# imkaywu/MVSKit

Measured on AMD Instinct MI355X. Metric: patches/s (propagate+optim iteration), 12-view 1080p, higher is better.
Workload: dtype f32

## Files before the change

### mvskit_amd/csrc/mvs_engine.cpp

```cpp
#include <dlfcn.h>

#include <cmath>
#include <cstring>

#include "mvs_engine_impl.h"

using namespace mvseng;

static_assert(sizeof(mvs_patch) == sizeof(DPatch), "mvs_patch and DPatch must be the same bytes");
static_assert((MVS_LISTCAP == 16 || MVS_LISTCAP == 32 || MVS_LISTCAP == 64) && MVS_LISTCAP <= MVS_MAXI && MVS_MAX_IMAGES == MVS_MAXI, "limits out of sync");

namespace mvseng {

thread_local std::string g_err;

Roctx& roctx() {
    static Roctx r;
    static bool tried = false;
    if (tried) return r;
    tried = true;
    void* h = nullptr;
    const char* names[] = {"libroctx64.so", "libroctx64.so.4", "/opt/rocm/lib/libroctx64.so.4"};
    for (const char* n : names) if (!h) h = dlopen(n, RTLD_NOW | RTLD_NOLOAD);
    for (const char* n : names) if (!h) h = dlopen(n, RTLD_NOW | RTLD_LOCAL);
    if (!h) return r;
    r.push = reinterpret_cast<int (*)(const char*)>(dlsym(h, "roctxRangePushA"));
    r.pop = reinterpret_cast<int (*)()>(dlsym(h, "roctxRangePop"));
    if (!r.push || !r.pop) { r.push = nullptr; r.pop = nullptr; }
    return r;
}

RefineSel refine_sel(const mvs_engine* e) {
    return RefineSel{e->refiner.mode == MVS_REFINE_CONVERGED ? 1 : 0, e->refiner.max_evals, e->refiner.xtol};
}

DParams current_params(mvs_engine* e) {
    DParams p = e->prm;
    p.views = e->dviews.p;
    p.pyr32 = e->pyr_narrow ? e->pyr.p : nullptr;
    p.pool = e->pool.p;
    p.pool_n = e->pool_n;
    p.total_cells = e->total_cells;
    p.csr_start = e->start.p; p.csr_cnt = e->cnt_alive.p; p.csr_key = e->key.p; p.csr_id32 = e->id32.p;
    p.vcsr_start = e->vstart.p; p.vcsr_cnt = e->vcnt_alive.p; p.vcsr_id32 = e->vid32.p;
    p.dpgrid = e->dpgrid.p;
    p.geo = e->geo_valid ? e->geo.p : nullptr;
    p.geo_ref = e->geo_valid ? e->geo_ref.p : nullptr;
    return p;
}

bool want_vgrid(const mvs_engine* e) { return e->prm.depth >= 2 && e->prm.enable_check; }

int need_state(const mvs_engine* e, Need need, const char* who) {
    if (!e) { g_err = std::string(who) + ": no engine"; return MVS_ERR_ARG; }
    if (need >= NEED_VIEWS && !e->have_views) { g_err = std::string(who) + ": views not set"; return MVS_ERR_STATE; }
    if (need >= NEED_IDLE && e->staged) { g_err = std::string(who) + ": a pass is waiting for its commit"; return MVS_ERR_STATE; }
    return MVS_OK;
}

int scan_total(mvs_engine* e, const int32_t* flags, int32_t* base, int32_t* scan, int64_t n, int64_t* count) {
    mvsk_exclusive_scan(flags, base, n, scan, e->stream);
    int32_t total = 0;
    if (int r = read_back(e, base + n, &total)) return r;
    HIPCHK(hipGetLastError());
    *count = total;
    return MVS_OK;
}

}

namespace {

void derive_params(mvs_engine* e) {
    const mvs_config& c = e->cfg;
    DParams& p = e->prm;
    p.nviews = c.nviews; p.level = c.level; p.csize = c.csize; p.wsize = c.wsize; p.wsz = c.wsize * c.wsize;
    p.minImageNum = c.minImageNum;
    p.tau = std::min(c.minImageNum * 2, c.nviews);
    p.max_propag = c.max_propag;
    p.cap = c.max_propag * c.csize * c.csize;
    p.depth = c.depth; p.enable_check = c.enable_check; p.view_propagation = c.view_propagation ? 1 : 0;
    p.seed = c.seed; p.refine_steps = c.refine_steps; p.rd0 = c.refine_rd0; p.ra0 = c.refine_ra0;
    p.nccThreshold = c.nccThreshold;
    p.nccThresholdBefore = c.nccThreshold - 0.3f;
    volatile float a0 = (float)(60.0f * M_PI / 180.0f), a1 = (float)(60.0f * M_PI / 180.0f);
    volatile double amin = (double)c.maxAngleThreshold, amax = (double)a1;
    volatile float typo = (float)(120.0f / M_PI * 180.0f);
    volatile double d120 = 120.0f * M_PI / 180.0f, d10 = 10.0f * M_PI / 180.0f;
    p.cosAngle0 = cosf(a0);
    p.cosAngle1 = cosf(a1);
    p.cosMinAngle = (float)cos(amin);
    p.cosMaxAngle = (float)cos(amax);
    p.cosNeighborTypo = cosf(typo);
    p.cosNeighbor120 = (float)cos(d120);
    p.sortThreshold = (float)(1.0f - cos(d10));
    p.ascaleConst = (float)(M_PI / 48.0f);
    p.inv_sz = 1.0f / (float)(c.wsize * c.wsize);
    p.inv_3sz = 1.0f / (float)(3 * c.wsize * c.wsize);
    p.neighborThreshold = 0.5f; p.neighborThreshold1 = 1.0f;
    p.quadThreshold = c.quadThreshold;
    p.list_n = std::min<int>(MVS_LISTCAP, c.nviews);
    p.gram_ld = (p.list_n + 15) / 16 * 16;
}

void invert3(const float* P, float* Minv) {
    double a = P[0], b = P[1], c = P[2], d = P[4], e = P[5], f = P[6], g = P[8], h = P[9], i = P[10];
    double A = e * i - f * h, B = -(d * i - f * g), C = d * h - e * g;
    double det = a * A + b * B + c * C;
    double inv[9] = {A, -(b * i - c * h), b * f - c * e, B, a * i - c * g, -(a * f - c * d), C, -(a * h - b * g), a * e - b * d};
    for (int k = 0; k < 9; ++k) Minv[k] = (float)(inv[k] / det);
}
inline float hfma(float a, float b, float c) { return __builtin_fmaf(a, b, c); }
inline float hdot3(const float* a, const float* b) { return hfma(a[2], b[2], hfma(a[1], b[1], a[0] * b[0])); }
inline float hdot4(const float* a, const float* b) { return hfma(a[3], b[3], hfma(a[2], b[2], hfma(a[1], b[1], a[0] * b[0]))); }
inline void hcross(const float* a, const float* b, float* o) {
    o[0] = a[1] * b[2] - a[2] * b[1]; o[1] = a[2] * b[0] - a[0] * b[2]; o[2] = a[0] * b[1] - a[1] * b[0];
}

void setup_camera(const mvs_engine* e, DView& vw, const float* P0) {
    const int maxLevel = e->cfg.level + 3;
    for (int k = 0; k < 12; ++k) vw.P[0][k] = P0[k];
    for (int l = 1; l < maxLevel; ++l) {
        for (int k = 0; k < 12; ++k) vw.P[l][k] = vw.P[l - 1][k];
        for (int k = 0; k < 8; ++k) vw.P[l][k] /= 2.0f;
    }
    invert3(vw.P[e->cfg.level], vw.Minv);
    const float* r2 = &vw.P[0][8];
    const float n = sqrtf(hdot3(r2, r2));
    for (int k = 0; k < 4; ++k) vw.oaxis[k] = r2[k] / n;
    {
        const float* P = vw.P[0];
        double a = P[0], b = P[1], c = P[2], d = P[4], ee = P[5], f = P[6], g = P[8], h = P[9], i = P[10];
        double A = ee * i - f * h, B = -(d * i - f * g), C = d * h - ee * g;
        double det = a * A + b * B + c * C;
        double inv[9] = {A, -(b * i - c * h), b * f - c * ee, B, a * i - c * g, -(a * f - c * d), C, -(a * h - b * g), a * ee - b * d};
        double q[3] = {P[3], P[7], P[11]};
        vw.center[0] = (float)(-(inv[0] * q[0] + inv[1] * q[1] + inv[2] * q[2]) / det);
        vw.center[1] = (float)(-(inv[3] * q[0] + inv[4] * q[1] + inv[5] * q[2]) / det);
        vw.center[2] = (float)(-(inv[6] * q[0] + inv[7] * q[1] + inv[8] * q[2]) / det);
        vw.center[3] = 1.0f;
    }
    for (int k = 0; k < 3; ++k) vw.zaxis[k] = vw.oaxis[k];
    float xa[3] = {vw.P[0][0], vw.P[0][1], vw.P[0][2]};
    hcross(vw.zaxis, xa, vw.yaxis);
    const float yn = sqrtf(hdot3(vw.yaxis, vw.yaxis));
    for (int k = 0; k < 3; ++k) vw.yaxis[k] /= yn;
    hcross(vw.yaxis, vw.zaxis, vw.xaxis);
    const float x4[4] = {vw.xaxis[0], vw.xaxis[1], vw.xaxis[2], 0.0f}, y4[4] = {vw.yaxis[0], vw.yaxis[1], vw.yaxis[2], 0.0f};
    vw.ipscale = hdot4(&vw.P[0][0], x4) + hdot4(&vw.P[0][4], y4);
}

}

extern "C" {

const char* mvs_last_error(void) { return g_err.c_str(); }

int mvs_list_cap(void) { return MVS_LISTCAP; }
int mvs_patch_bytes(void) { return (int)sizeof(mvs_patch); }

int mvs_device_count(void) {
    int n = 0;
    if (hipGetDeviceCount(&n) != hipSuccess) return 0;
    return n;
}

void mvs_default_refiner(mvs_refiner* r) {
    if (!r) return;
    r->mode = MVS_REFINE_HALVING; r->max_evals = 500; r->xtol = 1e-4f;
}

int mvs_engine_set_refiner(mvs_engine* e, const mvs_refiner* r) {
    if (!e || !r) { g_err = "mvs_engine_set_refiner: null argument"; return MVS_ERR_ARG; }
    if ((r->mode != MVS_REFINE_HALVING && r->mode != MVS_REFINE_CONVERGED) || r->max_evals < 5 || r->max_evals > 4096 ||
        !std::isfinite(r->xtol) || !(r->xtol > 0.0f)) {
        g_err = "mvs_engine_set_refiner: unknown mode, max_evals outside 5..4096, or xtol not finite and > 0";
        return MVS_ERR_ARG;
    }
    e->refiner = *r;
    return MVS_OK;
}

void mvs_default_config(mvs_config* c) {
    memset(c, 0, sizeof *c);
    c->level = 1; c->csize = 2; c->wsize = 7; c->minImageNum = 3; c->max_propag = 2;
    c->nccThreshold = 0.7f; c->maxAngleThreshold = (float)(10.0f * M_PI / 180.0f); c->quadThreshold = 2.5f;
    c->depth = 1; c->seed = 1; c->refine_steps = 6; c->refine_rd0 = 4.0f; c->refine_ra0 = 4.0f; c->enable_check = 1;
    c->view_begin = 0; c->view_stride = 1; c->device = 0; c->max_patches = 0;
}

int mvs_engine_create(const mvs_config* cfg, mvs_engine** out) {
    if (!cfg || !out) { g_err = "mvs_engine_create: null argument"; return MVS_ERR_ARG; }
    if (cfg->shard_count > 1 && (cfg->shard_index < 0 || cfg->shard_index >= cfg->shard_count)) { g_err = "mvs_engine_create: bad shard_index"; return MVS_ERR_ARG; }
    if (cfg->nviews < 1 || cfg->nviews > MVS_MAXVIEWS || cfg->wsize < 1 || cfg->wsize > 7 || cfg->csize < 1 || cfg->level < 0 ||
        cfg->level > 4 || cfg->max_propag < 1 || cfg->max_propag > 16 || cfg->max_propag * cfg->csize * cfg->csize > MVS_CAPMAX ||
        cfg->view_stride < 1 || cfg->view_begin < 0 || cfg->minImageNum < 1 ||
        std::min(cfg->minImageNum * 2, cfg->nviews) > 16 ) {
        g_err = "mvs_engine_create: configuration out of range (nviews <= 64, wsize <= 7, min(2 minImageNum, nviews) <= 16, max_propag*csize^2 <= 32)";
        return MVS_ERR_ARG;
    }
    int ndev = 0;
    if (hipGetDeviceCount(&ndev) != hipSuccess || ndev < 1) { g_err = "mvs_engine_create: no HIP device (the engine has no CPU path)"; return MVS_ERR_NO_DEVICE; }
    if (cfg->device < 0 || cfg->device >= ndev) { g_err = "mvs_engine_create: bad device ordinal"; return MVS_ERR_ARG; }
    HIPCHK(hipSetDevice(cfg->device));
    mvs_engine* e = new mvs_engine();
    e->cfg = *cfg;
    derive_params(e);
    hipError_t he = hipStreamCreate(&e->stream);
    if (he != hipSuccess) { g_err = std::string("hipStreamCreate: ") + hipGetErrorString(he); delete e; return MVS_ERR_HIP; }
    for (auto& ev : e->ev) (void)hipEventCreate(&ev);
    for (auto& ev : e->fev) (void)hipEventCreate(&ev);
    if (e->misc.ensure(misc::words) || e->counters.ensure(MVS_COUNTER_SLOTS) || e->error_flag.ensure(1)) { delete e; return MVS_ERR_HIP; }
    (void)hipMemset(e->misc.p, 0, misc::words * sizeof(unsigned long long));
    (void)hipMemset(e->error_flag.p, 0, sizeof(int32_t));
    *out = e;
    return MVS_OK;
}

int mvs_engine_destroy(mvs_engine* e) {
    if (!e) return MVS_OK;
    (void)hipSetDevice(e->cfg.device);
    (void)hipStreamSynchronize(e->stream);
    (void)mvs_engine_comm_release(e);
    for (auto& ev : e->ev) if (ev) (void)hipEventDestroy(ev);
    for (auto& ev : e->fev) if (ev) (void)hipEventDestroy(ev);
    (void)hipStreamDestroy(e->stream);
    delete e;
    return MVS_OK;
}

int mvs_engine_set_views(mvs_engine* e, int nviews, const mvs_view_desc* views) {
    if (!e || !views || nviews != e->cfg.nviews) { g_err = "mvs_engine_set_views: nviews must equal the configured number of views"; return MVS_ERR_ARG; }
    HIPCHK(hipSetDevice(e->cfg.device));
    hipStream_t st = e->stream;
    Range rg("mvs:set_views (upload + pyramids)");
    e->mask_bufs.clear();
    e->have_views = false;
    const int maxLevel = e->cfg.level + 3;
    e->hviews.assign(nviews, DView{});
    int cell_base = 0;
    size_t max_bytes = 0;
    for (int v = 0; v < nviews; ++v) {
        if (views[v].width < 8 || views[v].height < 8 || !views[v].rgb) { g_err = "mvs_engine_set_views: bad view"; return MVS_ERR_ARG; }
        max_bytes = std::max(max_bytes, (size_t)views[v].width * views[v].height * 3);
    }
    if (int r = e->tmp_bytes.ensure((int64_t)max_bytes)) return r;
    std::vector<uint64_t> level_off((size_t)nviews * maxLevel);
    uint64_t pyr_bytes = 0;
    bool narrow = true;
    for (int v = 0; v < nviews; ++v) {
        DView& vw = e->hviews[v];
        vw.W[0] = views[v].width; vw.H[0] = views[v].height;
        for (int l = 1; l < maxLevel; ++l) { vw.W[l] = vw.W[l - 1] / 2; vw.H[l] = vw.H[l - 1] / 2; }
        for (int l = 0; l < maxLevel; ++l) {
            level_off[(size_t)v * maxLevel + l] = pyr_bytes;
            pyr_bytes += (std::max<uint64_t>((uint64_t)vw.W[l] * vw.H[l], 1) * 4 + 255) / 256 * 256;
        }
        if ((int64_t)vw.W[0] * 4 >= (1 << 24) || vw.H[0] >= (1 << 24)) narrow = false;
    }
    if (pyr_bytes >= (1ull << 32)) narrow = false;
    if (int r = e->pyr.ensure((int64_t)pyr_bytes)) return r;
    e->pyr_narrow = narrow;
    for (int v = 0; v < nviews; ++v) {
        DView& vw = e->hviews[v];
        setup_camera(e, vw, views[v].P);
        const size_t n0 = (size_t)vw.W[0] * vw.H[0];
        HIPCHK(hipMemcpyAsync(e->tmp_bytes.p, views[v].rgb, n0 * 3, hipMemcpyHostToDevice, st));
        for (int l = 0; l < maxLevel; ++l) {
            const uint64_t off = level_off[(size_t)v * maxLevel + l];
            uint32_t* buf = reinterpret_cast<uint32_t*>(e->pyr.p + off);
            vw.img[l] = buf;
            vw.img_off[l] = (uint32_t)off;
            if (l == 0) mvsk_rgb_to_rgba(e->tmp_bytes.p, buf, (int64_t)n0, st);
            else mvsk_pyr_down(vw.img[l - 1], vw.W[l - 1], vw.H[l - 1], buf, vw.W[l], vw.H[l], st);
        }
        vw.mask = nullptr;
        if (views[v].mask) {
            HIPCHK(hipStreamSynchronize(st));
            uint8_t* prev = nullptr;
            for (int l = 0; l <= e->cfg.level; ++l) {
                e->mask_bufs.emplace_back();
                if (int r = e->mask_bufs.back().ensure(std::max<int64_t>((int64_t)vw.W[l] * vw.H[l], 1))) return r;
                uint8_t* m = e->mask_bufs.back().p;
                if (l == 0) {
                    HIPCHK(hipMemcpyAsync(m, views[v].mask, n0, hipMemcpyHostToDevice, st));
                    mvsk_mask_binarise(m, (int64_t)n0, st);
                } else mvsk_mask_down(prev, vw.W[l - 1], vw.H[l - 1], m, vw.W[l], vw.H[l], st);
                prev = m;
            }
            vw.mask = prev;
        }
        HIPCHK(hipStreamSynchronize(st));
        vw.gh = (vw.H[e->cfg.level] + e->cfg.csize - 1) / e->cfg.csize;
        vw.gw = (vw.W[e->cfg.level] + e->cfg.csize - 1) / e->cfg.csize;
        vw.cell_base = cell_base;
        cell_base += vw.gw * vw.gh;
    }
    e->total_cells = cell_base;
    if (int r = e->dviews.ensure(nviews)) return r;
    HIPCHK(hipMemcpyAsync(e->dviews.p, e->hviews.data(), sizeof(DView) * nviews, hipMemcpyHostToDevice, st));
    const int64_t nc = e->total_cells;
    if (e->cnt.ensure(nc + 2) || e->start.ensure(nc + 2) || e->cursor.ensure(nc + 2) || e->vcnt.ensure(nc + 2) || e->vstart.ensure(nc + 2) ||
        e->vcursor.ensure(nc + 2) || e->start_raw.ensure(nc + 2) || e->dpgrid.ensure(nc + 2) || e->best.ensure(nc + 2) || e->cnt_alive.ensure(nc + 2) || e->vcnt_alive.ensure(nc + 2))
        return MVS_ERR_HIP;
    int64_t pool_cap = e->cfg.max_patches > 0 ? e->cfg.max_patches : 4 * nc;
    if (e->cfg.max_patches <= 0) {
        size_t free_b = 0, total_b = 0;
        if (hipMemGetInfo(&free_b, &total_b) == hipSuccess && total_b > 0) {
            pool_cap = std::max<int64_t>(std::min<int64_t>(pool_cap, (int64_t)(total_b / 6 / sizeof(DPatch))), std::min<int64_t>(pool_cap, nc));
            const double per_patch = 2.5 * (double)sizeof(DPatch) + 17.0;
            const int64_t fit = (int64_t)(0.6 * (double)free_b / per_patch);
            if (fit < pool_cap) pool_cap = std::max<int64_t>(fit, std::min<int64_t>(pool_cap, nc / 4 + 1024));
        }
    }
    e->ids.headroom = e->key.headroom = e->id32.headroom = e->id32_raw.headroom = e->vid32.headroom = true;
    e->geo.headroom = e->geo_ref.headroom = true;
    if (e->pool.ensure(pool_cap) || e->pool_alt.ensure(pool_cap) || e->kill.ensure(pool_cap) || e->kill_cnt.ensure(pool_cap + 2) || e->kill_base.ensure(pool_cap + 2)) return MVS_ERR_HIP;
    HIPCHK(hipMemsetAsync(e->kill.p, 0, (size_t)pool_cap, st));
    int64_t njobs_max = 0;
    for (int v = 0; v < nviews; ++v) njobs_max += (int64_t)((e->hviews[v].gw + 1) / 2) * e->hviews[v].gh;
    const int maxstage = (e->prm.view_propagation ? 3 : 2) * e->prm.cap * e->prm.max_propag;
    if (e->job_stage.ensure(njobs_max * maxstage) || e->job_nstage.ensure(njobs_max + 2) || e->job_cnt.ensure(njobs_max + misc::job_list_pad) ||
        e->job_base_scan.ensure(njobs_max + misc::job_list_pad) || e->job_list.ensure(std::max<int64_t>(njobs_max, 16)))
        return MVS_ERR_HIP;
    const int64_t scan_n = std::max<int64_t>(std::max<int64_t>(nc, pool_cap), njobs_max);
    if (e->scan_tmp.ensure(scan_n / 256 + 4096)) return MVS_ERR_HIP;
    if (e->big_tables.ensure((int64_t)256 * 16384) || e->retry_jobs.ensure(std::max<int64_t>(njobs_max, 16))) return MVS_ERR_HIP;
    if (e->uf_parent.ensure(pool_cap) || e->uf_size.ensure(pool_cap) || e->dirty.ensure((nc + 31) / 32 + 1) || e->fstat_buf.ensure(fstat::words)) return MVS_ERR_HIP;
    if (e->staging.ensure(std::max<int64_t>(pool_cap / 2, 1024))) return MVS_ERR_HIP;
    if (e->tmp_rec_out.ensure(16)) return MVS_ERR_HIP;
    HIPCHK(hipStreamSynchronize(st));
    e->pool_n = 0;
    e->have_views = true;
    e->staged = false;
    return MVS_OK;
}

int mvs_engine_grid_dims(mvs_engine* e, int view, int* gw, int* gh) {
    if (!e || !e->have_views || view < 0 || view >= e->cfg.nviews) { g_err = "mvs_engine_grid_dims: bad view / views not set"; return MVS_ERR_STATE; }
    if (gw) *gw = e->hviews[view].gw;
    if (gh) *gh = e->hviews[view].gh;
    return MVS_OK;
}

int mvs_engine_get_pyramid(mvs_engine* e, int view, int level, uint8_t* rgb_out, int* W, int* H) {
    if (!e || !e->have_views || view < 0 || view >= e->cfg.nviews || level < 0 || level >= e->cfg.level + 3) { g_err = "mvs_engine_get_pyramid: bad argument"; return MVS_ERR_ARG; }
    HIPCHK(hipSetDevice(e->cfg.device));
    const DView& vw = e->hviews[view];
    if (W) *W = vw.W[level];
    if (H) *H = vw.H[level];
    if (!rgb_out) return MVS_OK;
    const int64_t n = (int64_t)vw.W[level] * vw.H[level];
    if (int r = e->tmp_bytes.ensure(n * 3)) return r;
    mvsk_rgba_to_rgb(vw.img[level], e->tmp_bytes.p, n, e->stream);
    HIPCHK(hipMemcpyAsync(rgb_out, e->tmp_bytes.p, (size_t)n * 3, hipMemcpyDeviceToHost, e->stream));
    HIPCHK(hipStreamSynchronize(e->stream));
    return MVS_OK;
}

int mvs_engine_set_thresholds(mvs_engine* e, float ncc, float before, int depth) {
    if (!e) return MVS_ERR_ARG;
    e->prm.nccThreshold = ncc; e->prm.nccThresholdBefore = before; e->prm.depth = depth;
    return MVS_OK;
}
int mvs_engine_get_thresholds(mvs_engine* e, float* ncc, float* before, int* depth) {
    if (!e) return MVS_ERR_ARG;
    if (ncc) *ncc = e->prm.nccThreshold;
    if (before) *before = e->prm.nccThresholdBefore;
    if (depth) *depth = e->prm.depth;
    return MVS_OK;
}
int mvs_engine_update_threshold(mvs_engine* e) {
    if (!e) return MVS_ERR_ARG;
    e->prm.nccThreshold -= 0.05f; e->prm.nccThresholdBefore -= 0.05f; ++e->prm.depth;
    return MVS_OK;
}

int mvs_engine_upload_patches(mvs_engine* e, int64_t n, const mvs_patch* patches) {
    if (!e || !e->have_views) { g_err = "mvs_engine_upload_patches: views not set"; return MVS_ERR_STATE; }
    if (n < 0 || (n > 0 && !patches)) return MVS_ERR_ARG;
    if (e->staged) { g_err = "mvs_engine_upload_patches: a pass is waiting for its commit"; return MVS_ERR_STATE; }
    HIPCHK(hipSetDevice(e->cfg.device));
    Range rg("mvs:upload_patches");
    std::vector<mvs_patch> recs;
    recs.reserve((size_t)n);
    for (int64_t i = 0; i < n; ++i) {
        mvs_patch p = patches[i];
        p.nimages = std::min(p.nimages, MVS_LISTCAP);
        if (p.nimages <= 0) continue;
        memset(p.images + p.nimages, 0, sizeof p.images - (size_t)p.nimages);
        p.nvimages = 0;
        memset(p.vimages, 0, sizeof p.vimages);
        p.tmp = std::max(0.0f, p.ncc - e->prm.nccThreshold) * p.nimages;
        p.flags = 1;
        p.id = 0;
        recs.push_back(p);
    }
    if (e->pool_n + (int64_t)recs.size() > e->pool.cap) { g_err = "mvs_engine_upload_patches: patch pool capacity exceeded (raise mvs_config.max_patches)"; return MVS_ERR_CAPACITY; }
    if (!recs.empty()) HIPCHK(hipMemcpyAsync(e->pool.p + e->pool_n, recs.data(), recs.size() * sizeof(mvs_patch), hipMemcpyHostToDevice, e->stream));
    HIPCHK(hipStreamSynchronize(e->stream));
    e->pool_n += (int64_t)recs.size();
    e->ncc_dirty = true;
    return MVS_OK;
}

int mvs_engine_reserve(mvs_engine* e, int64_t list_entries) {
    if (!e || !e->have_views || list_entries < 0) { g_err = "mvs_engine_reserve: views not set, or a negative size"; return MVS_ERR_ARG; }
    HIPCHK(hipSetDevice(e->cfg.device));
    int64_t n = list_entries > 0 ? list_entries : e->total_cells * (int64_t)(e->cfg.max_propag * e->cfg.csize * e->cfg.csize);
    auto take = [&](auto& buf, int64_t want) -> int {
        const int64_t before = buf.cap;
        if (int r = buf.ensure(want)) return r;
        if (buf.cap != before && hipMemsetAsync(buf.p, 0, (size_t)buf.cap * sizeof(*buf.p), e->stream) != hipSuccess) { (void)hipGetLastError(); return MVS_ERR_HIP; }
        return MVS_OK;
    };
    if (take(e->ids, n + 16) || take(e->key, n + 16) || take(e->id32, n + 16) || take(e->id32_raw, n + 16) || take(e->vid32, n + 16)) return MVS_ERR_HIP;
    HIPCHK(hipStreamSynchronize(e->stream));
    return MVS_OK;
}

int mvs_engine_clear_patches(mvs_engine* e) {
    if (!e) return MVS_ERR_ARG;
    HIPCHK(hipSetDevice(e->cfg.device));
    if (e->kill.p) HIPCHK(hipMemsetAsync(e->kill.p, 0, (size_t)e->kill.cap, e->stream));
    e->pool_n = 0; e->staged = false; e->counted = false;
    return MVS_OK;
}

int mvs_engine_num_patches(mvs_engine* e, int64_t* n_alive) {
    if (!e || !n_alive) return MVS_ERR_ARG;
    HIPCHK(hipSetDevice(e->cfg.device));
    return count_pool(e, Count::alive, n_alive);
}

int mvs_engine_download_patches(mvs_engine* e, int64_t cap, mvs_patch* out, int64_t* n) {
    if (!e || !n) return MVS_ERR_ARG;
    int64_t alive = 0;
    if (int r = mvs_engine_num_patches(e, &alive)) return r;
    *n = alive;
    if (!out || alive == 0) return MVS_OK;
    const int64_t m = std::min(cap, alive);
    if (int r = e->tmp_rec_out.ensure(alive)) return r;
    mvsk_alive_gather(e->pool.p, e->pool_n, e->kill_base.p, e->tmp_rec_out.p, alive, e->stream);
    HIPCHK(hipMemcpyAsync(out, e->tmp_rec_out.p, (size_t)m * sizeof(mvs_patch), hipMemcpyDeviceToHost, e->stream));
    HIPCHK(hipStreamSynchronize(e->stream));
    return MVS_OK;
}

int mvs_engine_sweep_pairs(mvs_engine* e, int64_t out[6]) {
    if (!e || !out) return MVS_ERR_ARG;
    for (int k = 0; k < 6; ++k) out[k] = e->sweep_pairs[k];
    return MVS_OK;
}

int mvs_engine_sweep_repeats(mvs_engine* e, int64_t out[2]) {
    if (!e || !out) return MVS_ERR_ARG;
    for (int k = 0; k < 2; ++k) out[k] = e->sweep_repeats[k];
    return MVS_OK;
}

int mvs_engine_sweep_kernels(mvs_engine* e, int64_t out[2]) {
    if (!e || !out) return MVS_ERR_ARG;
    for (int k = 0; k < 2; ++k) out[k] = e->sweep_kernels[k];
    return MVS_OK;
}

int mvs_engine_sampler_launches(mvs_engine* e, int64_t out[4]) {
    if (!e || !out) return MVS_ERR_ARG;
    for (int k = 0; k < 4; ++k) out[k] = e->sampler_launches[k];
    return MVS_OK;
}

int mvs_engine_last_timing(mvs_engine* e, mvs_timing* t) {
    if (!e || !t) return MVS_ERR_ARG;
    *t = e->timing;
    return MVS_OK;
}

int mvs_engine_depth_normal_map(mvs_engine* e, int view, int kind, float* depth, float* normal, int32_t* ids) {
    if (!e || !e->have_views || view < 0 || view >= e->cfg.nviews || kind < 0 || kind > 1) { g_err = "mvs_engine_depth_normal_map: bad argument"; return MVS_ERR_ARG; }
    HIPCHK(hipSetDevice(e->cfg.device));
    hipStream_t st = e->stream;
    const DView& vw = e->hviews[view];
    const int ncells = vw.gw * vw.gh;
    const DParams p = current_params(e);
    const unsigned long long* sel = nullptr;
    if (kind == 0) {
        HIPCHK(hipMemsetAsync(e->dpgrid.p, 0xff, (size_t)e->total_cells * sizeof(unsigned long long), st));
        mvsk_depth_maps(p, e->dpgrid.p, nullptr, st);
        sel = e->dpgrid.p + vw.cell_base;
    } else {
        HIPCHK(hipMemsetAsync(e->best.p, 0, (size_t)ncells * sizeof(unsigned long long), st));
        mvsk_best_ncc_map(p, view, e->best.p, st);
        sel = e->best.p;
    }
    if (e->tmp_f_out.ensure((int64_t)ncells * 4) || e->tmp_i.ensure(ncells)) return MVS_ERR_HIP;
    mvsk_map_extract(p, view, kind, sel, e->tmp_f_out.p, e->tmp_f_out.p + ncells, e->tmp_i.p, ncells, st);
    if (depth) HIPCHK(hipMemcpyAsync(depth, e->tmp_f_out.p, (size_t)ncells * sizeof(float), hipMemcpyDeviceToHost, st));
    if (normal) HIPCHK(hipMemcpyAsync(normal, e->tmp_f_out.p + ncells, (size_t)ncells * 3 * sizeof(float), hipMemcpyDeviceToHost, st));
    if (ids) HIPCHK(hipMemcpyAsync(ids, e->tmp_i.p, (size_t)ncells * sizeof(int32_t), hipMemcpyDeviceToHost, st));
    HIPCHK(hipStreamSynchronize(st));
    return MVS_OK;
}

int mvs_engine_probe(mvs_engine* e, int op, int64_t n, const mvs_patch* in_rec, const float* in_f, mvs_patch* out_rec, float* out_f, int32_t* out_i) {
    if (!e || !e->have_views || n < 0 || op < 0 || op > 6) { g_err = "mvs_engine_probe: bad argument / views not set"; return MVS_ERR_ARG; }
    const RefineSel rs = refine_sel(e);
    if (op == MVS_PROBE_REFINE_X && !rs.simplex) { g_err = "mvs_engine_probe: MVS_PROBE_REFINE_X needs the CONVERGED refiner"; return MVS_ERR_STATE; }
    if (n == 0) return MVS_OK;
    HIPCHK(hipSetDevice(e->cfg.device));
    hipStream_t st = e->stream;
    if (op == MVS_PROBE_POSTPROCESS && e->prm.depth > 0) if (int r = build_index(e, nullptr)) return r;
    const int64_t nf_out = op == MVS_PROBE_MATH ? 5 * n : ((op == MVS_PROBE_REFINE || op == MVS_PROBE_REFINE_X) && rs.simplex ? 4 * n : n);
    if (e->tmp_rec_in.ensure(n) || e->tmp_rec_out.ensure(n) || e->tmp_f_in.ensure(n) || e->tmp_f_out.ensure(nf_out) || e->tmp_i.ensure(n + 1)) return MVS_ERR_HIP;
    if (op == MVS_PROBE_MATH) {
        if (!in_f || !out_f) return MVS_ERR_ARG;
        HIPCHK(hipMemcpyAsync(e->tmp_f_in.p, in_f, (size_t)n * sizeof(float), hipMemcpyHostToDevice, st));
    } else {
        if (!in_rec) return MVS_ERR_ARG;
        HIPCHK(hipMemcpyAsync(e->tmp_rec_in.p, in_rec, (size_t)n * sizeof(mvs_patch), hipMemcpyHostToDevice, st));
    }
    HIPCHK(hipMemsetAsync(e->tmp_i.p, 0, (size_t)(n + 1) * sizeof(int32_t), st));
    const DParams p = current_params(e);
    const KernelVariant probe_kernel = mvsk_probe(p, op, n, e->tmp_rec_in.p, e->tmp_f_in.p, e->tmp_rec_out.p, e->tmp_f_out.p, e->tmp_i.p, rs, st);
    if (probe_kernel.launched) e->sampler_launches[probe_kernel.narrow ? 3 : 2] += 1;
    if (out_rec && (op == MVS_PROBE_PREPROCESS || op == MVS_PROBE_REFINE || op == MVS_PROBE_POSTPROCESS || op == MVS_PROBE_REFINE_X))
        HIPCHK(hipMemcpyAsync(out_rec, e->tmp_rec_out.p, (size_t)n * sizeof(mvs_patch), hipMemcpyDeviceToHost, st));
    if (out_f && (op == MVS_PROBE_NCC || op == MVS_PROBE_COST || op == MVS_PROBE_MATH || op == MVS_PROBE_REFINE_X))
        HIPCHK(hipMemcpyAsync(out_f, e->tmp_f_out.p, (size_t)nf_out * sizeof(float), hipMemcpyDeviceToHost, st));
    if (out_i) HIPCHK(hipMemcpyAsync(out_i, e->tmp_i.p, (size_t)n * sizeof(int32_t), hipMemcpyDeviceToHost, st));
    HIPCHK(hipStreamSynchronize(st));
    HIPCHK(hipGetLastError());
    return MVS_OK;
}

}
```

### mvskit_amd/csrc/mvs_engine_impl.h

```cpp
#pragma once
#include <hip/hip_runtime.h>
#include <rccl/rccl.h>

#include <algorithm>
#include <cstdint>
#include <string>
#include <vector>

#include "mvskit_engine.h"
#include "mvs_kernels.h"
#include "mvs_types.h"

namespace mvseng {
extern thread_local std::string g_err;
}

#define HIPCHK(expr)                                                                                       \
    do {                                                                                                   \
        hipError_t _e = (expr);                                                                            \
        if (_e != hipSuccess) {                                                                            \
            mvseng::g_err = std::string(#expr) + ": " + hipGetErrorString(_e);                             \
            return MVS_ERR_HIP;                                                                            \
        }                                                                                                  \
    } while (0)

#define MVS_XCHG_WORDS 5

namespace mvseng {

template <typename T> struct DevBuf {
    T* p = nullptr;
    int64_t cap = 0;
    bool headroom = false;
    DevBuf() = default;
    DevBuf(const DevBuf&) = delete;
    DevBuf(DevBuf&& o) noexcept : p(o.p), cap(o.cap), headroom(o.headroom) { o.p = nullptr; o.cap = 0; }
    ~DevBuf() { release(); }
    void swap(DevBuf& o) { std::swap(p, o.p); std::swap(cap, o.cap); }
    int ensure(int64_t n) {
        if (n <= cap) return MVS_OK;
        const int64_t exact = std::max<int64_t>(n, 16);
        int64_t want = (p && headroom) ? exact + exact / 2 : exact;
        T* q = nullptr;
        hipError_t e = hipMalloc((void**)&q, (size_t)want * sizeof(T));
        if (e != hipSuccess && want > exact) { (void)hipGetLastError(); want = exact; e = hipMalloc((void**)&q, (size_t)want * sizeof(T)); }
        if (e != hipSuccess && p) {
            (void)hipGetLastError();
            (void)hipFree(p); p = nullptr; cap = 0;
            e = hipMalloc((void**)&q, (size_t)want * sizeof(T));
        }
        if (e != hipSuccess) { (void)hipGetLastError(); g_err = std::string("hipMalloc: ") + hipGetErrorString(e); return MVS_ERR_HIP; }
        if (p) (void)hipFree(p);
        p = q; cap = want;
        return MVS_OK;
    }
    void release() { if (p) (void)hipFree(p); p = nullptr; cap = 0; }
};

namespace misc {
constexpr int stage_counter = 0;
constexpr int fill_evals = 1;
constexpr int neighbor_retry = 4;
constexpr int sweep_retry = 5;
constexpr int geo_bad = 6;
constexpr int group_edges = 7;
constexpr int trim_parts = 8;
constexpr int trim_nparts = 256;
constexpr int sweep_cursors = (trim_parts + trim_nparts + 15) / 16 * 16;
constexpr int sweep_cursor_words = MVS_SWEEP_QUEUES * MVS_SWEEP_CURSOR_STRIDE * (int)sizeof(uint32_t) / (int)sizeof(unsigned long long);
constexpr int sweep_list_bounds = sweep_cursors + sweep_cursor_words;
constexpr int sweep_list_bound_words = (MVS_SWEEP_QUEUES + 1 + 1) / 2;
constexpr int words = sweep_list_bounds + sweep_list_bound_words;
constexpr int64_t job_list_pad = 1024 + 2;
}
namespace fstat {
constexpr int neighbor_parts = 0;
constexpr int neighbor_cycles = 4096;
constexpr int exact_evals = 4112;
constexpr int words = exact_evals + 2048;
}

struct Rccl {
    void* h = nullptr;
    ncclResult_t (*GetUniqueId)(ncclUniqueId*) = nullptr;
    ncclResult_t (*CommInitRank)(ncclComm_t*, int, ncclUniqueId, int) = nullptr;
    ncclResult_t (*CommDestroy)(ncclComm_t) = nullptr;
    ncclResult_t (*CommCount)(const ncclComm_t, int*) = nullptr;
    ncclResult_t (*CommUserRank)(const ncclComm_t, int*) = nullptr;
    ncclResult_t (*AllGather)(const void*, void*, size_t, ncclDataType_t, ncclComm_t, hipStream_t) = nullptr;
    ncclResult_t (*Broadcast)(const void*, void*, size_t, ncclDataType_t, int, ncclComm_t, hipStream_t) = nullptr;
    ncclResult_t (*GroupStart)() = nullptr;
    ncclResult_t (*GroupEnd)() = nullptr;
    const char* (*GetErrorString)(ncclResult_t) = nullptr;
    bool ok = false;
};
Rccl& rccl();

struct Roctx {
    int (*push)(const char*) = nullptr;
    int (*pop)() = nullptr;
};
Roctx& roctx();
struct Range {
    bool on;
    explicit Range(const char* name) : on(roctx().push != nullptr) { if (on) roctx().push(name); }
    ~Range() { if (on) roctx().pop(); }
    Range(const Range&) = delete;
    Range& operator=(const Range&) = delete;
};

}

using mvseng::DevBuf;
struct mvs_engine {
    mvs_config cfg{};
    mvs_refiner refiner{MVS_REFINE_HALVING, 500, 1e-4f};
    DParams prm{};
    hipStream_t stream = nullptr;
    bool have_views = false;
    std::vector<DView> hviews;
    DevBuf<DView> dviews;
    DevBuf<uint8_t> pyr;
    bool pyr_narrow = false;
    std::vector<DevBuf<uint8_t>> mask_bufs;
    int total_cells = 0;
    DevBuf<DPatch> pool, pool_alt;
    DevBuf<uint8_t> kill;
    int64_t pool_n = 0;
    bool ncc_dirty = false;
    DevBuf<int32_t> cnt, cursor, vcnt, vcursor;
    DevBuf<csr_off_t> start, vstart;
    DevBuf<csr_off_t> start_raw;
    DevBuf<int32_t> id32_raw;
    DevBuf<int64_t> scan_tmp;
    DevBuf<unsigned long long> ids;
    DevBuf<ListKey> key;
    DevBuf<int32_t> id32, vid32;
    DevBuf<int32_t> uf_parent, uf_size;
    DevBuf<int32_t> group_edges;
    DevBuf<int32_t> cnt_alive, vcnt_alive;
    DevBuf<unsigned long long> dpgrid, best;
    DevBuf<uint32_t> dirty;
    bool dirty_marked = false;
    DevBuf<float4> geo;
    DevBuf<uint8_t> geo_ref;
    bool geo_valid = false;
    bool lists_dense[2] = {false, false};
    DevBuf<DPatch> staging;
    DevBuf<int32_t> job_stage, job_nstage, job_cnt, job_base_scan, kill_cnt, kill_base;
    DevBuf<unsigned long long> misc;
    DevBuf<DCounters> counters;
    DevBuf<int32_t> error_flag;
    DevBuf<int32_t> big_tables, retry_jobs;
    DevBuf<int32_t> job_list;
    int64_t sweep_pairs[6] = {0, 0, 0, 0, 0, 0};
    int64_t sweep_repeats[2] = {0, 0};
    int64_t sweep_kernels[2] = {0, 0};
    int64_t sampler_launches[4] = {0, 0, 0, 0};
    int64_t retried_cells = 0;
    int64_t pass_retried = 0;
    SweepArgs sa{};
    bool staged = false;
    bool counted = false;
    int64_t n_new = 0, n_kill = 0;
    std::vector<int32_t> h_per_view;
    DevBuf<DPatch> tmp_rec_in, tmp_rec_out;
    DevBuf<float> tmp_f_in, tmp_f_out;
    DevBuf<int32_t> tmp_i;
    DevBuf<uint8_t> tmp_bytes;
    hipEvent_t ev[6] = {nullptr, nullptr, nullptr, nullptr, nullptr, nullptr};
    mvs_timing timing{};
    mvs_filter_stats fstats{};
    int64_t fstats_exchange_bytes = 0;
    DevBuf<unsigned long long> fstat_buf;
    hipEvent_t fev[10] = {nullptr, nullptr, nullptr, nullptr, nullptr, nullptr, nullptr, nullptr, nullptr, nullptr};
    ncclComm_t comm = nullptr;
    bool comm_owned = false;
    int comm_rank = 0, comm_world = 1;
    DevBuf<int64_t> comm_counts;
    DevBuf<int32_t> comm_kill_ids;
    int pass_status = MVS_OK;
    std::string pass_error;
    bool fault_fired = false;
};

namespace mvseng {

RefineSel refine_sel(const mvs_engine* e);
DParams current_params(mvs_engine* e);
bool want_vgrid(const mvs_engine* e);
enum Need { NEED_ENGINE, NEED_VIEWS, NEED_IDLE };
int need_state(const mvs_engine* e, Need need, const char* who);
int scan_total(mvs_engine* e, const int32_t* flags, int32_t* base, int32_t* scan, int64_t n, int64_t* count);

int build_list(mvs_engine* e, bool vgrid, bool trim, bool unordered = false);
int build_depth(mvs_engine* e);
int build_index(mvs_engine* e, unsigned long long* trimmed_out);
enum class Count { alive, kills, apply_kills };
int count_pool(mvs_engine* e, Count what, int64_t* total);
int ensure_counts(mvs_engine* e);
int compact_pool(mvs_engine* e);
void discard_pass(mvs_engine* e);

template <typename T> int read_back(mvs_engine* e, const T* dev, T* host) {
    HIPCHK(hipMemcpyAsync(host, dev, sizeof(T), hipMemcpyDeviceToHost, e->stream));
    HIPCHK(hipStreamSynchronize(e->stream));
    return MVS_OK;
}

template <typename Apply> int commit_pool(mvs_engine* e, Apply&& apply) {
    hipStream_t st = e->stream;
    HIPCHK(hipEventRecord(e->ev[2], st));
    int64_t n_new = 0;
    if (int r = apply(&n_new)) return r;
    e->pool_n += n_new;
    if (int r = compact_pool(e)) return r;
    HIPCHK(hipEventRecord(e->ev[3], st));
    HIPCHK(hipStreamSynchronize(st));
    float ms = 0.0f;
    (void)hipEventElapsedTime(&ms, e->ev[2], e->ev[3]);
    e->timing.commit_ms = ms;
    e->staged = false; e->counted = false;
    return MVS_OK;
}

template <typename Blocks> ncclResult_t broadcast_blocks(mvs_engine* e, Blocks&& blocks) {
    const Rccl& R = rccl();
    ncclResult_t first = R.GroupStart();
    for (int r = 0; r < e->comm_world && first == ncclSuccess; ++r)
        blocks(r, [&](void* p, int64_t n, ncclDataType_t type) {
            if (n > 0 && first == ncclSuccess) first = R.Broadcast(p, p, (size_t)n, type, r, e->comm, e->stream);
        });
    const ncclResult_t end = R.GroupEnd();
    return first == ncclSuccess ? end : first;
}

struct MapsBufs {
    MapsArgs args{};
    int64_t total_pix = 0, max_pix = 0;
    DevBuf<int32_t> ids;
    DevBuf<float> pts;
    DevBuf<unsigned long long> agree;
    DevBuf<int32_t> flag, base, scan;
    DevBuf<float> maps;
    DevBuf<uint8_t> flag8;
    DevBuf<mvs_fused_point> recs;
};
int maps_args(const mvs_maps_config* c, const char* who);
int maps_state(const mvs_engine* e, const mvs_maps_config* c, const char* who);
int64_t maps_npix(const mvs_engine* e, int v);
int render_all(mvs_engine* e, const mvs_maps_config* c, MapsBufs& b);
int render_usable(mvs_engine* e, const mvs_maps_config* c, MapsBufs& b);

}
```

### mvskit_amd/csrc/mvs_engine_pass.cpp

```cpp
#include <climits>
#include <cstdio>
#include <cstdlib>
#include <cstring>

#include "mvs_engine_impl.h"

using namespace mvseng;

namespace mvseng {

int build_list(mvs_engine* e, bool vgrid, bool trim, bool unordered) {
    hipStream_t st = e->stream;
    const int64_t nc = e->total_cells;
    DParams p = current_params(e);
    DevBuf<int32_t>& cnt = vgrid ? e->vcnt : e->cnt;
    DevBuf<csr_off_t>& start = vgrid ? e->vstart : e->start;
    DevBuf<int32_t>& cursor = vgrid ? e->vcursor : e->cursor;
    DevBuf<unsigned long long>& ids = e->ids;
    DevBuf<int32_t>& id32 = vgrid ? e->vid32 : e->id32;
    DevBuf<int32_t>& cnt_alive = vgrid ? e->vcnt_alive : e->cnt_alive;
    HIPCHK(hipMemsetAsync(cnt.p, 0, (size_t)(nc + 1) * sizeof(int32_t), st));
    mvsk_index_count(p, vgrid ? nullptr : cnt.p, vgrid ? cnt.p : nullptr, nullptr, st);
    const bool direct = unordered && !trim;
    DevBuf<csr_off_t>& raw = e->start_raw;
    csr_off_t* const first_scan = direct ? start.p : raw.p;
    mvsk_exclusive_scan_off(cnt.p, first_scan, nc, reinterpret_cast<csr_off_t*>(e->scan_tmp.p), st);
    csr_off_t tot64 = 0;
    if (int r = read_back(e, first_scan + nc, &tot64)) return r;
    const int64_t tot = (int64_t)tot64;
    if (!unordered) { if (int r = ids.ensure(tot + 16)) return r; }
    if (!vgrid && !unordered) { if (int r = e->key.ensure(tot + 16)) return r; }
    if (int r = id32.ensure(tot + 16)) return r;
    p = current_params(e);
    HIPCHK(hipMemsetAsync(cursor.p, 0, (size_t)(nc + 1) * sizeof(int32_t), st));
    if (direct) {
        mvsk_index_fill_direct(p, vgrid ? 1 : 0, start.p, cursor.p, id32.p, st);
        cnt.swap(cnt_alive);
        e->lists_dense[vgrid ? 1 : 0] = true;
        return MVS_OK;
    }
    if (int r = e->id32_raw.ensure(tot + 16)) return r;
    mvsk_index_fill(p, vgrid ? 1 : 0, raw.p, cursor.p, ids.p, st);
    mvsk_index_sort_trim(p, raw.p, ids.p, trim ? 1 : 0, e->misc.p + misc::trim_parts, st);
    mvsk_index_finalize(p, vgrid ? 1 : 0, raw.p, ids.p, e->id32_raw.p, cnt_alive.p, st);
    mvsk_exclusive_scan_off(cnt_alive.p, start.p, nc, reinterpret_cast<csr_off_t*>(e->scan_tmp.p), st);
    mvsk_index_pack(p, raw.p, start.p, cnt_alive.p, ids.p, e->id32_raw.p, vgrid ? nullptr : e->key.p, id32.p, st);
    e->lists_dense[vgrid ? 1 : 0] = true;
    return MVS_OK;
}
int build_depth(mvs_engine* e) {
    const DParams p = current_params(e);
    HIPCHK(hipMemsetAsync(e->dpgrid.p, 0xff, (size_t)e->total_cells * sizeof(unsigned long long), e->stream));
    mvsk_depth_maps(p, e->dpgrid.p, nullptr, e->stream);
    return MVS_OK;
}
int build_index(mvs_engine* e, unsigned long long* trimmed_out) {
    hipStream_t st = e->stream;
    const DParams p = current_params(e);
    HIPCHK(hipMemsetAsync(e->misc.p + misc::fill_evals, 0, 2 * sizeof(unsigned long long), st));
    HIPCHK(hipMemsetAsync(e->misc.p + misc::trim_parts, 0, misc::trim_nparts * sizeof(unsigned long long), st));
    mvsk_fill_ncc(p, e->misc.p + misc::fill_evals, st);
    e->ncc_dirty = false;
    if (int r = build_list(e, false, true)) return r;
    if (want_vgrid(e)) if (int r = build_list(e, true, false, true)) return r;
    if (int r = build_depth(e)) return r;
    if (trimmed_out) {
        unsigned long long part[misc::trim_nparts];
        HIPCHK(hipMemcpyAsync(part, e->misc.p + misc::trim_parts, sizeof part, hipMemcpyDeviceToHost, st));
        HIPCHK(hipStreamSynchronize(st));
        *trimmed_out = 0;
        for (unsigned long long v : part) *trimmed_out += v;
    }
    HIPCHK(hipGetLastError());
    return MVS_OK;
}

int count_pool(mvs_engine* e, Count what, int64_t* total) {
    hipStream_t st = e->stream;
    *total = 0;
    if (e->pool_n == 0) return MVS_OK;
    if (what == Count::alive) mvsk_alive_count(e->pool.p, e->pool_n, e->kill_cnt.p, st);
    else mvsk_kill_count(e->kill.p, e->pool_n, e->kill_cnt.p, st);
    mvsk_exclusive_scan(e->kill_cnt.p, e->kill_base.p, e->pool_n, reinterpret_cast<int32_t*>(e->scan_tmp.p), st);
    int32_t n = 0;
    HIPCHK(hipMemcpyAsync(&n, e->kill_base.p + e->pool_n, sizeof n, hipMemcpyDeviceToHost, st));
    if (what == Count::apply_kills) mvsk_apply_kill_flags(e->pool.p, e->kill.p, e->pool_n, st);
    HIPCHK(hipStreamSynchronize(st));
    *total = n;
    return MVS_OK;
}

int ensure_counts(mvs_engine* e) {
    if (e->counted) return MVS_OK;
    hipStream_t st = e->stream;
    const int64_t nj = e->sa.njobs;
    e->n_new = 0; e->n_kill = 0;
    e->h_per_view.assign(e->cfg.nviews, 0);
    if (nj > 0) {
        mvsk_commit_count(e->sa, e->job_cnt.p, st);
        mvsk_exclusive_scan(e->job_cnt.p, e->job_base_scan.p, nj, reinterpret_cast<int32_t*>(e->scan_tmp.p), st);
        std::vector<int32_t> bounds(e->sa.nsweep_views + 1);
        for (int s = 0; s < e->sa.nsweep_views; ++s)
            HIPCHK(hipMemcpyAsync(&bounds[s], e->job_base_scan.p + e->sa.job_base[s], sizeof(int32_t), hipMemcpyDeviceToHost, st));
        HIPCHK(hipMemcpyAsync(&bounds[e->sa.nsweep_views], e->job_base_scan.p + nj, sizeof(int32_t), hipMemcpyDeviceToHost, st));
        HIPCHK(hipStreamSynchronize(st));
        e->n_new = bounds[e->sa.nsweep_views];
        for (int s = 0; s < e->sa.nsweep_views; ++s) e->h_per_view[e->sa.sweep_views[s]] = bounds[s + 1] - bounds[s];
    }
    if (int r = count_pool(e, Count::kills, &e->n_kill)) return r;
    e->counted = true;
    return MVS_OK;
}

int compact_pool(mvs_engine* e) {
    int64_t alive = 0;
    if (int r = count_pool(e, Count::alive, &alive)) return r;
    if (alive == e->pool_n) return MVS_OK;
    mvsk_alive_gather(e->pool.p, e->pool_n, e->kill_base.p, e->pool_alt.p, e->pool_alt.cap, e->stream);
    e->pool.swap(e->pool_alt);
    e->pool_n = alive;
    return MVS_OK;
}

void discard_pass(mvs_engine* e) {
    if (e->kill.p && e->pool_n > 0) (void)hipMemsetAsync(e->kill.p, 0, (size_t)e->pool_n, e->stream);
    (void)hipStreamSynchronize(e->stream);
    e->staged = false; e->counted = false;
}

}

namespace {

template <typename C> void add_counters(mvs_counters& a, const C& b) {
    a.candidates += b.candidates; a.prefiltered += b.prefiltered; a.patches += b.patches; a.fail0 += b.fail0; a.fail1 += b.fail1;
    a.inserted += b.inserted; a.replaced += b.replaced; a.evals += b.evals; a.view_evals += b.view_evals; a.trimmed += b.trimmed;
}

}

extern "C" {

static int pass_impl(mvs_engine* e, int iter, int pass, mvs_counters* out);
int mvs_engine_pass(mvs_engine* e, int iter, int pass, mvs_counters* out) {
    const int r = pass_impl(e, iter, pass, out);
    if (e) { e->pass_status = r; e->pass_error = r ? g_err : std::string(); }
    return r;
}
static int pass_impl(mvs_engine* e, int iter, int pass, mvs_counters* out) {
    if (!e || !e->have_views) { g_err = "mvs_engine_pass: views not set"; return MVS_ERR_STATE; }
    if (e->staged) { g_err = "mvs_engine_pass: the previous pass was not committed"; return MVS_ERR_STATE; }
    HIPCHK(hipSetDevice(e->cfg.device));
    hipStream_t st = e->stream;
    HIPCHK(hipEventRecord(e->ev[0], st));
    unsigned long long trimmed = 0;
    {
        Range rg("mvs:index");
        if (int r = build_index(e, &trimmed)) return r;
    }
    SweepArgs& a = e->sa;
    memset(&a, 0, sizeof a);
    a.iter = iter; a.inc = (iter % 2 == 0) ? 1 : -1; a.colour = pass & 1;
    int64_t nj = 0;
    const bool ranged = e->cfg.shard_count > 1;
    for (int v = ranged ? 0 : e->cfg.view_begin; v < e->cfg.nviews; v += ranged ? 1 : e->cfg.view_stride) {
        a.sweep_views[a.nsweep_views] = v;
        a.job_base[a.nsweep_views] = (int32_t)nj;
        ++a.nsweep_views;
        nj += (int64_t)((e->hviews[v].gw + 1) / 2) * e->hviews[v].gh;
    }
    a.njobs = nj;
    a.job_lo = 0; a.job_hi = nj;
    if (ranged) {
        const int split_mode = getenv("MVS_SPLIT_PROXY") ? atoi(getenv("MVS_SPLIT_PROXY")) : 2;
        const int N = e->cfg.shard_count, R = e->cfg.shard_index;
        std::vector<int32_t> cuts(N + 1, -1);
        int64_t total_work = 0;
        if (split_mode > 0 && nj > 0) {
            const DParams p0 = current_params(e);
            int shift = 0;
            while ((((int64_t)3 * e->prm.cap * e->prm.max_propag * 32 * nj) >> shift) + nj >= (int64_t)INT32_MAX) ++shift;
            mvsk_job_work(p0, a, split_mode, shift, e->job_cnt.p, st);
            mvsk_exclusive_scan(e->job_cnt.p, e->job_base_scan.p, nj, reinterpret_cast<int32_t*>(e->scan_tmp.p), st);
            if (int r = e->tmp_i.ensure(N + 1)) return r;
            HIPCHK(hipMemsetAsync(e->tmp_i.p, 0xff, (size_t)(N + 1) * sizeof(int32_t), st));
            mvsk_job_cuts(e->job_base_scan.p, nj, N, e->tmp_i.p, st);
            int32_t tw = 0;
            HIPCHK(hipMemcpyAsync(cuts.data(), e->tmp_i.p, (size_t)(N + 1) * sizeof(int32_t), hipMemcpyDeviceToHost, st));
            HIPCHK(hipMemcpyAsync(&tw, e->job_base_scan.p + nj, sizeof tw, hipMemcpyDeviceToHost, st));
            HIPCHK(hipStreamSynchronize(st));
            total_work = tw;
        }
        cuts[0] = 0; cuts[N] = (int32_t)nj;
        for (int r = 1; r < N; ++r) {
            if (total_work <= 0 || cuts[r] < 0) cuts[r] = (int32_t)(nj * r / N);
            cuts[r] = std::max(cuts[r], cuts[r - 1]);
        }
        a.job_lo = cuts[R];
        a.job_hi = cuts[R + 1];
    }
    a.staging = e->staging.p; a.staging_cap = e->staging.cap;
    a.stage_counter = e->misc.p + misc::stage_counter;
    a.job_stage = e->job_stage.p; a.job_nstage = e->job_nstage.p;
    a.maxstage = (e->prm.view_propagation ? 3 : 2) * e->prm.cap * e->prm.max_propag;
    a.kill = e->kill.p;
    a.counters = e->counters.p;
    a.error_flag = e->error_flag.p;
    if (want_vgrid(e)) {
        if (int r = e->big_tables.ensure((int64_t)256 * 16384)) return r;
        if (int r = e->retry_jobs.ensure(std::max<int64_t>(nj, 16))) return r;
    }
    a.big_tables = e->big_tables.p; a.retry_jobs = e->retry_jobs.p; a.nretry = reinterpret_cast<int32_t*>(e->misc.p + misc::sweep_retry);
    HIPCHK(hipMemsetAsync(e->misc.p + misc::sweep_retry, 0, sizeof(unsigned long long), st));
    HIPCHK(hipMemsetAsync(e->misc.p + misc::stage_counter, 0, sizeof(unsigned long long), st));
    a.cursors = reinterpret_cast<uint32_t*>(e->misc.p + misc::sweep_cursors);
    HIPCHK(hipMemsetAsync(e->misc.p + misc::sweep_cursors, 0, (misc::sweep_cursor_words + misc::sweep_list_bound_words) * sizeof(unsigned long long), st));
    HIPCHK(hipMemsetAsync(e->counters.p, 0, MVS_COUNTER_SLOTS * sizeof(DCounters), st));
    HIPCHK(hipMemsetAsync(e->error_flag.p, 0, sizeof(int32_t), st));
    const DParams p = current_params(e);
    const RefineSel rs = refine_sel(e);
    if (int r = e->job_list.ensure(std::max<int64_t>(nj, 16))) return r;
    if (e->job_cnt.ensure(nj + misc::job_list_pad) || e->job_base_scan.ensure(nj + misc::job_list_pad)) return MVS_ERR_HIP;
    int32_t* list_bounds = reinterpret_cast<int32_t*>(e->misc.p + misc::sweep_list_bounds);
    a.job_list = e->job_list.p; a.list_bounds = list_bounds;
    mvsk_job_list(p, a, e->job_cnt.p, e->job_base_scan.p, reinterpret_cast<int32_t*>(e->scan_tmp.p), e->job_list.p, list_bounds, st);
    HIPCHK(hipEventRecord(e->ev[1], st));
    Range rg_sweep(pass & 1 ? "mvs:sweep colour 1" : "mvs:sweep colour 0");
    const KernelVariant sweep_kernel = mvsk_sweep(p, a, rs, st);
    if (sweep_kernel.launched) { e->sweep_kernels[sweep_kernel.full_window ? 1 : 0] += 1; e->sampler_launches[sweep_kernel.narrow ? 1 : 0] += 1; }
    e->pass_retried = 0;
    if (want_vgrid(e)) {
        int32_t nretry = 0;
        if (int r = read_back(e, a.nretry, &nretry)) return r;
        e->pass_retried = nretry;
        if (nretry > 0) { mvsk_sweep_retry(p, a, nretry, rs, st); e->retried_cells += nretry; }
    }
    HIPCHK(hipEventRecord(e->ev[2], st));
    std::vector<DCounters> hcs(MVS_COUNTER_SLOTS);
    int32_t herr = 0;
    unsigned long long fill[2] = {0, 0};
    HIPCHK(hipMemcpyAsync(fill, e->misc.p + misc::fill_evals, sizeof fill, hipMemcpyDeviceToHost, st));
    HIPCHK(hipMemcpyAsync(hcs.data(), e->counters.p, hcs.size() * sizeof(DCounters), hipMemcpyDeviceToHost, st));
    HIPCHK(hipMemcpyAsync(&herr, e->error_flag.p, sizeof herr, hipMemcpyDeviceToHost, st));
    int32_t hbounds[MVS_SWEEP_QUEUES + 1];
    HIPCHK(hipMemcpyAsync(hbounds, list_bounds, sizeof hbounds, hipMemcpyDeviceToHost, st));
    HIPCHK(hipStreamSynchronize(st));
    HIPCHK(hipGetLastError());
    mvs_counters sum{};
    for (const DCounters& c : hcs) {
        add_counters(sum, c);
        for (int k = 0; k < 6; ++k) e->sweep_pairs[k] += (int64_t)c.pair[k];
        for (int k = 0; k < 2; ++k) e->sweep_repeats[k] += (int64_t)c.repeats[k];
    }
    sum.evals += fill[0]; sum.view_evals += fill[1]; sum.trimmed = (int64_t)trimmed;
    float ms = 0.0f;
    (void)hipEventElapsedTime(&ms, e->ev[0], e->ev[1]); e->timing.index_ms = ms;
    (void)hipEventElapsedTime(&ms, e->ev[1], e->ev[2]); e->timing.sweep_ms = ms;
    e->timing.commit_ms = 0.0f; e->timing.sweep_launches = 1; e->timing.exchange_ms = 0.0f; e->timing.exchange_bytes = 0;
    e->timing.check_retried_cells = e->pass_retried;
    e->timing.sweep_jobs_listed = hbounds[MVS_SWEEP_QUEUES];
    e->staged = true; e->counted = false;
    if (out) *out = sum;
#ifdef MVS_JOBLIST_COUNTS
    fprintf(stderr, "[job list] iter %d colour %d: jobs %lld, with any source entry %llu, listed %llu\n", iter, pass & 1, (long long)(a.job_hi - a.job_lo),
            hcs[0].stage[0], hcs[0].stage[1]);
#endif
#ifdef MVS_STAGE_TIMING
    {
        unsigned long long stage[16] = {0};
        for (const DCounters& c : hcs)
            for (int k = 0; k < 16; ++k) stage[k] = (k == 12 || k == 13) ? std::max(stage[k], c.stage[k]) : stage[k] + c.stage[k];
        static const char* nm[8] = {"wave", "generate", "pre", "refine", "post", "check", "stage", "prologue"};
        fprintf(stderr, "[stage cycles]");
        for (int k = 0; k < 8; ++k) fprintf(stderr, " %s %.1f%%", nm[k], 100.0 * (double)stage[k] / (double)(stage[0] ? stage[0] : 1));
        static const char* nm2[4] = {"gain", "search", "sort", "quad"};
        for (int k = 0; k < 4; ++k) fprintf(stderr, " %s %.1f%%", nm2[k], 100.0 * (double)stage[8 + k] / (double)(stage[0] ? stage[0] : 1));
        fprintf(stderr, " setRefImage pairs %.1f%% choice %.1f%%", 100.0 * (double)stage[14] / (double)(stage[0] ? stage[0] : 1), 100.0 * (double)stage[15] / (double)(stage[0] ? stage[0] : 1));
        fprintf(stderr, "  (wave cycles %.3e; max visited %llu, max neighbours %llu)\n", (double)stage[0], stage[12], stage[13]);
    }
#endif
#ifdef MVS_FAULT_INJECTION
    if (const char* f = getenv("MVS_FAULT_PASS")) {
        int fr = -1, fi = -1, fp = -1;
        if (!e->fault_fired && sscanf(f, "%d:%d:%d", &fr, &fi, &fp) == 3 && fr == (e->cfg.shard_count > 1 ? e->cfg.shard_index : 0) && fi == iter && fp == pass) {
            e->fault_fired = true;
            g_err = "mvs_engine_pass: capacity failure injected by MVS_FAULT_PASS";
            return MVS_ERR_CAPACITY;
        }
    }
#endif
    if (herr & 3) { g_err = "mvs_engine_pass: staging capacity exceeded (raise mvs_config.max_patches)"; return MVS_ERR_CAPACITY; }
    if (herr & 4) {
        g_err = "mvs_engine_pass: Optim::check met more than 14336 patches around one patch, or more than 4064 neighbours (engine limit)";
        return MVS_ERR_CAPACITY;
    }
    return MVS_OK;
}

int mvs_engine_export_counts(mvs_engine* e, int64_t* n_new, int64_t* n_kill, int32_t* per_view_new) {
    if (!e || !e->staged) { g_err = "mvs_engine_export_counts: no pass to export"; return MVS_ERR_STATE; }
    HIPCHK(hipSetDevice(e->cfg.device));
    if (int r = ensure_counts(e)) return r;
    if (n_new) *n_new = e->n_new;
    if (n_kill) *n_kill = e->n_kill;
    if (per_view_new) for (int v = 0; v < e->cfg.nviews; ++v) per_view_new[v] = e->h_per_view[v];
    return MVS_OK;
}

int mvs_engine_export_device(mvs_engine* e, void* d_new, int64_t cap_new, void* d_kill, int64_t cap_kill) {
    if (!e || !e->staged) { g_err = "mvs_engine_export_device: no pass to export"; return MVS_ERR_STATE; }
    HIPCHK(hipSetDevice(e->cfg.device));
    if (int r = ensure_counts(e)) return r;
    if (e->n_new > cap_new || e->n_kill > cap_kill) { g_err = "mvs_engine_export_device: buffers too small"; return MVS_ERR_CAPACITY; }
    if (e->n_new > 0) mvsk_commit_copy(e->sa, e->job_base_scan.p, (DPatch*)d_new, cap_new, nullptr, 1, e->stream);
    if (e->n_kill > 0) mvsk_kill_export(e->kill.p, e->pool_n, e->kill_base.p, (int32_t*)d_kill, cap_kill, e->stream);
    HIPCHK(hipStreamSynchronize(e->stream));
    return MVS_OK;
}

int mvs_engine_commit_device(mvs_engine* e, const void* d_new, int64_t n_new, const void* d_kill, int64_t n_kill) {
    if (!e || !e->have_views) return MVS_ERR_STATE;
    HIPCHK(hipSetDevice(e->cfg.device));
    hipStream_t st = e->stream;
    if (e->pool_n + n_new > e->pool.cap) { g_err = "mvs_engine_commit_device: patch pool capacity exceeded (raise mvs_config.max_patches)"; return MVS_ERR_CAPACITY; }
    return commit_pool(e, [&](int64_t* added) -> int {
        mvsk_apply_kill_ids(e->pool.p, (const int32_t*)d_kill, n_kill, e->pool_n, st);
        mvsk_append_records(e->pool.p, e->pool_n, (const DPatch*)d_new, n_new, st);
        if (e->pool_n > 0) HIPCHK(hipMemsetAsync(e->kill.p, 0, (size_t)e->pool_n, st));
        *added = n_new;
        return MVS_OK;
    });
}

int mvs_engine_commit_local(mvs_engine* e) {
    if (!e || !e->staged) { g_err = "mvs_engine_commit_local: no pass to commit"; return MVS_ERR_STATE; }
    HIPCHK(hipSetDevice(e->cfg.device));
    hipStream_t st = e->stream;
    Range rg("mvs:commit");
    return commit_pool(e, [&](int64_t* added) -> int {
        if (int r = ensure_counts(e)) return r;
        if (e->pool_n + e->n_new > e->pool.cap) { g_err = "mvs_engine_commit_local: patch pool capacity exceeded (raise mvs_config.max_patches)"; return MVS_ERR_CAPACITY; }
        if (e->n_new > 0) mvsk_commit_copy(e->sa, e->job_base_scan.p, e->pool.p + e->pool_n, e->pool.cap - e->pool_n, nullptr, 0, st);
        mvsk_apply_kill_flags(e->pool.p, e->kill.p, e->pool_n, st);
        *added = e->n_new;
        return MVS_OK;
    });
}

int mvs_engine_propagate(mvs_engine* e, int iter, mvs_counters* out) {
    mvs_counters total;
    memset(&total, 0, sizeof total);
    mvs_timing tt{};
    for (int pass = 0; pass < 2; ++pass) {
        mvs_counters c;
        memset(&c, 0, sizeof c);
        const int rp = mvs_engine_pass(e, iter, pass, &c);
        if (e && e->comm) {
            if (int r = mvs_engine_exchange(e)) return r;
        } else {
            if (rp) { if (e && e->staged) { const std::string keep = g_err; discard_pass(e); g_err = keep; } return rp; }
            if (int r = mvs_engine_commit_local(e)) return r;
        }
        add_counters(total, c);
        tt.index_ms += e->timing.index_ms; tt.sweep_ms += e->timing.sweep_ms; tt.commit_ms += e->timing.commit_ms; tt.sweep_launches += 1;
        tt.exchange_ms += e->timing.exchange_ms; tt.exchange_bytes += e->timing.exchange_bytes; tt.check_retried_cells += e->timing.check_retried_cells;
        tt.sweep_jobs_listed += e->timing.sweep_jobs_listed;
    }
    e->timing = tt;
    if (out) *out = total;
    return MVS_OK;
}

}
```

### mvskit_amd/csrc/mvs_filter.cuh

```cuda
#pragma once
#include <hip/hip_runtime.h>
#include <algorithm>
#include "mvs_patch_common.cuh"
#include "mvs_check.cuh"
#include "mvs_kernels.h"

using namespace mvsdev;

__global__ __launch_bounds__(64) void k_fill_ncc(DParams prm, unsigned long long* evals) {
    WaveCtx wc = make_wave_ctx(prm);
    const int64_t mine = (int64_t)blockIdx.x * 64 + wc.lane;
    bool need = false;
    if (mine < prm.pool_n) need = (prm.pool[mine].flags & 1) && (prm.pool[mine].ncc < 0.0f);
    unsigned long long todo = ballot(need);
    while (todo) {
        const int l = __ffsll((long long)todo) - 1;
        todo &= todo - 1ull;
        DPatch* p = prm.pool + ((int64_t)blockIdx.x * 64 + l);
        Cand c;
        load_cand(p, wc, c);
        const float ncc = compute_ncc(prm, wc, c.coord, c.normal, c.img, c.nimg);
        if (wc.lane == 0) p->ncc = ncc;
    }
    if (wc.lane == 0 && wc.evals) { atomicAdd(evals, (unsigned long long)wc.evals); atomicAdd(evals + 1, (unsigned long long)wc.view_evals); }
}
__global__ void k_kill_count(const uint8_t* __restrict__ kill, int64_t n, int32_t* __restrict__ cnt) {
    const int64_t i = (int64_t)blockIdx.x * blockDim.x + threadIdx.x;
    if (i < n) cnt[i] = kill[i] ? 1 : 0;
}
__global__ void k_kill_export(const uint8_t* __restrict__ kill, int64_t n, const int32_t* __restrict__ base, int32_t* __restrict__ ids, int64_t cap) {
    const int64_t i = (int64_t)blockIdx.x * blockDim.x + threadIdx.x;
    if (i < n && kill[i] && base[i] < cap) ids[base[i]] = (int32_t)i;
}
__global__ void k_apply_kill_flags(DPatch* pool, uint8_t* kill, int64_t n) {
    const int64_t i = (int64_t)blockIdx.x * blockDim.x + threadIdx.x;
    if (i < n && kill[i]) { pool[i].flags &= ~1; kill[i] = 0; }
}
__global__ void k_apply_kill_ids(DPatch* pool, const int32_t* __restrict__ ids, int64_t n, int64_t pool_n) {
    const int64_t i = (int64_t)blockIdx.x * blockDim.x + threadIdx.x;
    if (i < n && ids[i] >= 0 && ids[i] < pool_n) pool[ids[i]].flags &= ~1;
}
__global__ void k_append_records(DPatch* pool, int64_t pool_n, const DPatch* __restrict__ recs, int64_t n) {
    const int64_t i = (int64_t)blockIdx.x * blockDim.x + threadIdx.x;
    if (i >= n) return;
    const uint4* s4 = reinterpret_cast<const uint4*>(recs + i);
    uint4* d4 = reinterpret_cast<uint4*>(pool + pool_n + i);
    for (int w = 0; w < (int)MVS_REC_U4; ++w) d4[w] = s4[w];
    pool[pool_n + i].flags = 1;
    pool[pool_n + i].id = 0;
}
__global__ void k_alive_count(const DPatch* __restrict__ pool, int64_t n, int32_t* __restrict__ cnt) {
    const int64_t i = (int64_t)blockIdx.x * blockDim.x + threadIdx.x;
    if (i < n) cnt[i] = pool[i].flags & 1;
}
__global__ void k_alive_gather(const DPatch* __restrict__ pool, int64_t n, const int32_t* __restrict__ base, DPatch* __restrict__ out, int64_t cap) {
    const int64_t i = (int64_t)blockIdx.x * blockDim.x + threadIdx.x;
    if (i >= n || !(pool[i].flags & 1) || base[i] >= cap) return;
    const uint4* s4 = reinterpret_cast<const uint4*>(pool + i);
    uint4* d4 = reinterpret_cast<uint4*>(out + base[i]);
    for (int w = 0; w < (int)MVS_REC_U4; ++w) d4[w] = s4[w];
    out[base[i]].id = (int32_t)i;
}

DEV void set_vgrids(const DParams& prm, const WaveCtx& wc, Cand& c) {
    c.vgx = 0; c.vgy = 0;
    if (wc.lane < c.nvimg) cell_of(prm, prm.views + c.vimg, c.coord, c.vgx, c.vgy);
}
DEV void store_lists(DPatch* p, const WaveCtx& wc, const Cand& c) {
    if (wc.lane == 0) { p->nimages = c.nimg; p->nvimages = c.nvimg; }
    if (wc.lane < MVS_MAXI) {
        p->images[wc.lane] = (uint8_t)(wc.lane < c.nimg ? c.img : 0);
        p->vimages[wc.lane] = (uint8_t)(wc.lane < c.nvimg ? c.vimg : 0);
    }
}
template <int GL>
__global__ __launch_bounds__(64) void k_filter_vimages(DParams prm, int additive, int64_t first, int64_t last, const uint32_t* __restrict__ dirty) {
    __shared__ int s_new[64];
    const int lane = (int)threadIdx.x, g = lane / GL, i = lane % GL;
    const int64_t id = first + (int64_t)blockIdx.x * (64 / GL) + g;
    const bool have = id < last;
    DPatch* p = prm.pool + (have ? id : first);
    const bool act = have && (p->flags & 1);
    const int nimg = act ? min(p->nimages, MVS_LISTCAP) : 0;
    const int nv0 = act && additive ? min(p->nvimages, MVS_LISTCAP) : 0;
    const int my_img = i < MVS_MAXI ? (int)p->images[i] : 0, my_vimg = i < MVS_MAXI ? (int)p->vimages[i] : 0;
    unsigned long long listed = (i < nimg ? 1ull << my_img : 0ull) | (i < nv0 ? 1ull << my_vimg : 0ull);
#pragma unroll
    for (int d = 1; d < GL; d <<= 1) {
        const unsigned lo = (unsigned)__shfl_xor((int)(unsigned)listed, d), hi = (unsigned)__shfl_xor((int)(unsigned)(listed >> 32), d);
        listed |= ((unsigned long long)hi << 32) | lo;
    }
    bool q = false;
    if (act && i < prm.nviews && !((listed >> i) & 1ull)) {
        Cand c;
        c.coord = ld4(p->coord); c.normal = ld4(p->normal);
        int ix, iy;
        const DView* vw = prm.views + i;
        cell_of(prm, vw, c.coord, ix, iy);
        bool test = true;
        if (dirty && !(ix < 0 || vw->gw <= ix || iy < 0 || vw->gh <= iy)) { const int cell = vw->cell_base + iy * vw->gw + ix; test = (dirty[cell >> 5] >> (cell & 31)) & 1u; }
        q = test && is_visible(prm, c, i, ix, iy, prm.neighborThreshold) != 0;
    }
    const unsigned long long all = __ballot(q);
    const unsigned long long gm = GL == 64 ? all : (all >> (GL * g)) & ((1ull << (GL & 63)) - 1ull);
    const int added = (int)__popcll(gm), pos = (int)__popcll(gm & ((1ull << i) - 1ull));
    if (q) s_new[GL * g + pos] = i;
    __syncthreads();
    const int nv = min(MVS_LISTCAP, nv0 + added);
    if (act) {
        if (i == 0) { p->nimages = nimg; p->nvimages = nv; }
        if (i < MVS_MAXI) {
            p->images[i] = (uint8_t)(i < nimg ? my_img : 0);
            p->vimages[i] = (uint8_t)(i < nv0 ? my_vimg : (i < nv ? s_new[GL * g + (i - nv0)] : 0));
        }
        for (int k = i + GL; k < MVS_MAXI; k += GL) { p->images[k] = 0; p->vimages[k] = 0; }
    }
}
__global__ __launch_bounds__(64) void k_filter_outside(DParams prm, uint8_t* kill, int64_t first) {
    __shared__ int s_dummy[1];
    __shared__ int s_gain[MVS_LISTCAP];
    const int64_t pid = first + (int64_t)blockIdx.x;
    const DPatch* p = prm.pool + pid;
    if (!(p->flags & 1)) return;
    WaveCtx wc = make_wave_ctx(prm);
    Cand c;
    load_cand(p, wc, c);
    set_grids(prm, wc, c);
    set_vgrids(prm, wc, c);
    const CheckCtx cx{prm.pool, -1, -1, 0, s_dummy, nullptr};
    const float gain = prm.geo ? compute_gain<true>(prm, wc, cx, c, s_gain) : compute_gain<false>(prm, wc, cx, c, s_gain);
    if (wc.lane == 0 && gain < 0.0f) kill[pid] = 1;
}
__global__ void k_geo_pack(const DPatch* pool, int64_t n, float4* geo, uint8_t* ref, int* bad) {
    const int64_t i = (int64_t)blockIdx.x * blockDim.x + threadIdx.x;
    if (i >= n) return;
    const DPatch* p = pool + i;
    const F4 c = ld4(p->coord), nr = ld4(p->normal);
    geo[2 * i] = make_float4(c.x, c.y, c.z, p->dscale);
    geo[2 * i + 1] = make_float4(nr.x, nr.y, nr.z, p->ncc);
    ref[i] = p->images[0];
    if ((p->flags & 1) && !(c.w == 1.0f && nr.w == 0.0f)) *bad = 1;
}
#define MVS_FE_LANES (MVS_LISTCAP <= 16 ? 16 : (MVS_LISTCAP <= 32 ? 32 : 64))
#define MVS_FE_PATCHES (64 / MVS_FE_LANES)
__global__ __launch_bounds__(64) void k_filter_exact(DParams prm, uint8_t* kill, unsigned long long* evals, unsigned long long* stage, int64_t first, int64_t last) {
    __shared__ int s_scratch[192];
    extern __shared__ float s_texs[];
    WaveCtx wc = make_wave_ctx(prm);
#ifdef MVS_STAGE_TIMING
    const unsigned long long fe_begin = (unsigned long long)__builtin_amdgcn_s_memtime();
    WC_T0(wc)
#endif
    const int q = wc.lane / MVS_FE_LANES, i = wc.lane % MVS_FE_LANES;
    const int64_t id = first + (int64_t)blockIdx.x * MVS_FE_PATCHES + q;
    const bool have = id < last;
    const DPatch* pl = prm.pool + (have ? id : 0);
    const bool alive_l = have && (pl->flags & 1);
    const int nimg_l = alive_l ? min(pl->nimages, MVS_LISTCAP) : 0;
    const bool act = i < nimg_l;
    const int image = act ? (int)pl->images[i] : 0;
    const F4 coord = ld4(pl->coord), normal = ld4(pl->normal);
    WC_ADD(wc, 5)
    bool safe = false;
    {
        const DView* vw = prm.views + image;
        const int w = vw->gw, h = vw->gh, cbase = vw->cell_base;
        const F4 ctr = ld4(vw->center);
        const float ips = vw->ipscale;
        int x, y;
        cell_of(prm, vw, coord, x, y);
        const bool in = act && !(x < 0 || w <= x || y < 0 || h <= y);
        const int dxs[5] = {0, -1, 1, 0, 0}, dys[5] = {0, 0, 0, -1, 1};
        bool ok[5];
        unsigned long long dp[5];
#pragma unroll
        for (int k = 0; k < 5; ++k) {
            const int xx = x + dxs[k], yy = y + dys[k];
            ok[k] = in && 0 <= xx && xx < w && 0 <= yy && yy < h;
            dp[k] = prm.dpgrid[cbase + (ok[k] ? yy * w + xx : 0)];
        }
        F4 qc[5];
#pragma unroll
        for (int k = 0; k < 5; ++k) qc[k] = ld4((prm.pool + (dp[k] == ~0ull ? 0u : (uint32_t)(dp[k] & 0xffffffffull)))->coord);
        const F4 ray = nrm4(sub4(coord, ctr));
        const float factor = fminf(2.0f, 2.0f + dot4(ray, normal));
        float unit = 1.0f;
        if (ips != 0.0f) unit = (2.0f * norm4(sub4(coord, ctr)) * (float)(1 << prm.level)) / ips;
        const float rhs = (unit * (float)prm.csize * prm.neighborThreshold1) * factor;
#pragma unroll
        for (int k = 0; k < 5; ++k) {
            const float diff = dot4(ray, sub4(coord, qc[k]));
            const bool vis = prm.depth == 0 || dp[k] == ~0ull || diff < rhs;
            safe |= ok[k] && vis;
        }
    }
    WC_ADD(wc, 6)
    const unsigned long long safe_b = ballot(safe);
    const unsigned long long alive_b = ballot(alive_l);
    const int tstride = prm.wsz;
    Frame fpre = {};
    {
        const unsigned long long gbits = MVS_FE_LANES == 64 ? ~0ull : ((1ull << (MVS_FE_LANES & 63)) - 1ull) << ((MVS_FE_LANES * q) & 63);
        const bool skip_l = (pl->flags & MVS_FLAG_SETTLED) && (int)__popcll(safe_b & gbits) == nimg_l;
        if (ballot(alive_l && !skip_l)) {
            int vmin = safe ? image : INT_MAX;
            for (int d = 1; d < MVS_FE_LANES; d <<= 1) vmin = min(vmin, __shfl_xor(vmin, d));
            F4 px, py;
            get_paxes(prm, prm.views + (vmin == INT_MAX ? 0 : vmin), coord, normal, px, py);
            fpre = make_frame(prm, coord, px, py, normal, image, safe);
        }
    }
    WC_ADD(wc, 1)
    for (int g = 0; g < MVS_FE_PATCHES; ++g) {
        if (!((alive_b >> ((MVS_FE_LANES * g) & 63)) & 1ull)) continue;
        DPatch* p = prm.pool + (first + (int64_t)blockIdx.x * MVS_FE_PATCHES + g);
        const int pflags = p->flags;
        Cand c;
        load_cand(p, wc, c);
        const vmask_t sm = (vmask_t)((safe_b >> ((MVS_FE_LANES * g) & 63)) & (MVS_FE_LANES == 64 ? ~0ull : (1ull << (MVS_FE_LANES & 63)) - 1ull));
        if ((pflags & MVS_FLAG_SETTLED) && (int)vpop(sm) == c.nimg) continue;
        __syncthreads();
        if (wc.lane < MVS_MAXVIEWS) s_scratch[wc.lane] = 0;
        __syncthreads();
        if (wc.lane < c.nimg && ((sm >> wc.lane) & 1u)) s_scratch[c.img] = 1 + MVS_FE_LANES * g + wc.lane;
        __syncthreads();
        const int src1 = s_scratch[wc.lane];
        const bool present = src1 != 0;
        const unsigned long long pm = ballot(present);
        const int pos = __popcll(pm & ((1ull << wc.lane) - 1ull));
        __syncthreads();
        if (present && pos < MVS_LISTCAP) { s_scratch[64 + pos] = wc.lane; s_scratch[128 + pos] = src1 - 1; }
        __syncthreads();
        c.nimg = min((int)__popcll(pm), MVS_LISTCAP);
        c.img = s_scratch[64 + wc.lane];
        if (prm.minImageNum <= c.nimg) {
            Frame f;
            {
                const bool mine = wc.lane < c.nimg;
                const int src = mine ? s_scratch[128 + wc.lane] : MVS_FE_LANES * g;
                f.tlx = __shfl(fpre.tlx, src); f.tly = __shfl(fpre.tly, src);
                f.dxx = __shfl(fpre.dxx, src); f.dxy = __shfl(fpre.dxy, src); f.dyx = __shfl(fpre.dyx, src); f.dyy = __shfl(fpre.dyy, src);
                f.w = __shfl(fpre.w, src); f.ok = __shfl(fpre.ok, src);
                f.a_lo = (unsigned)__shfl((int)fpre.a_lo, src); f.a_hi = (unsigned)__shfl((int)fpre.a_hi, src);
                if (!mine) { f.tlx = f.tly = f.dxx = f.dxy = f.dyx = f.dyy = 0.0f; f.ok = 0; }
            }
            WC_ADD(wc, 7)
            set_ref_image(prm, wc, s_texs, tstride, c, nullptr, &f);
            store_lists(p, wc, c);
            if (wc.lane == 0) p->flags = pflags | MVS_FLAG_SETTLED;
            WC_ADD(wc, 7)
        } else {
            if (wc.lane == 0) kill[first + (int64_t)blockIdx.x * MVS_FE_PATCHES + g] = 1;
        }
    }
    if (wc.lane == 0 && wc.evals) { atomicAdd(evals + 2 * (blockIdx.x & 1023u), (unsigned long long)wc.evals); atomicAdd(evals + 2 * (blockIdx.x & 1023u) + 1, (unsigned long long)wc.view_evals); }
#ifdef MVS_STAGE_TIMING
    if (stage && wc.lane == 0) {
        atomicAdd(stage, (unsigned long long)__builtin_amdgcn_s_memtime() - fe_begin);
        for (int k = 1; k < 8; ++k) atomicAdd(stage + k, wc.st_acc[k]);
    }
#endif
}
template <int HCAP, int RCAP>
__global__ __launch_bounds__(64) void k_filter_neighbor(DParams prm, uint8_t* kill, const int32_t* todo, int32_t ntodo, int32_t* retry, int32_t* nretry,
                                                        int32_t* overflow, unsigned long long* stats , int64_t first) {
    extern __shared__ float s_lds[];
    int* const s_dummy = reinterpret_cast<int*>(s_lds);
    const int64_t id = todo ? (blockIdx.x < (unsigned)ntodo ? todo[blockIdx.x] : -1) : first + (int64_t)blockIdx.x;
    if (id < 0 || id >= prm.pool_n) return;
    const DPatch* p = prm.pool + id;
    if (!(p->flags & 1)) return;
    WaveCtx wc = make_wave_ctx(prm);
#ifdef MVS_STAGE_TIMING
    unsigned long long st_acc[16] = {0, 0, 0, 0, 0, 0, 0, 0, 0, 0, 0, 0, 0, 0, 0, 0};
    const unsigned long long st_begin = CK_NOW();
    auto st_flush = [&]() { st_acc[0] = CK_NOW() - st_begin; if (wc.lane == 0) for (int k = 0; k < 12; ++k) if (st_acc[k]) atomicAdd(stats + 4096 + k, st_acc[k]); };
#endif
    Cand c;
    load_cand(p, wc, c);
    set_grids(prm, wc, c);
#ifdef MVS_STAGE_TIMING
    const CheckCtx cx{prm.pool, -1, -1, 0, s_dummy, st_acc};
    st_acc[1] = CK_NOW() - st_begin;
#else
    const CheckCtx cx{prm.pool, -1, -1, 0, s_dummy, nullptr};
#endif
    int* table = reinterpret_cast<int*>(s_lds);
    unsigned st4[4] = {0u, 0u, 0u, 0u};
    const bool pk = prm.geo != nullptr;
    constexpr bool MK = HCAP == MVS_FILTER_HASH_CAP;
    int* const marks = reinterpret_cast<int*>(s_lds) + MVS_SET_LDS_FLOATS(HCAP, RCAP);
    const int n = pk ? find_neighbors<HCAP, false, true, MK>(prm, wc, cx, c, table, 4.0f, 2, st4, marks) : find_neighbors<HCAP, false, false, MK>(prm, wc, cx, c, table, 4.0f, 2, st4, marks);
    if (n < 0 || n > RCAP) {
        if (wc.lane == 0) {
            if (retry) retry[atomicAdd(nretry, 1)] = (int32_t)id;
            else atomicOr(overflow, 4);
        }
#ifdef MVS_STAGE_TIMING
        st_flush();
#endif
        return;
    }
    if (wc.lane < 4) atomicAdd(stats + 4 * (blockIdx.x & 1023u) + wc.lane, (unsigned long long)(wc.lane == 0 ? st4[0] : wc.lane == 1 ? st4[1] : wc.lane == 2 ? st4[2] : st4[3]));
    const bool reject = n < 6 || (pk ? filter_quad<false, true>(prm, wc, cx, c, table, n, s_lds + rows_offset(n)) : filter_quad<false, false>(prm, wc, cx, c, table, n, s_lds + rows_offset(n))) != 0;
    if (wc.lane == 0 && reject) kill[id] = 1;
#ifdef MVS_STAGE_TIMING
    st_acc[11] = CK_NOW() - st_begin - st_acc[1] - st_acc[9] - st_acc[10];
    st_flush();
#endif
}
__global__ void k_groups_init(int* parent, int* size, int64_t n) {
    const int64_t i = (int64_t)blockIdx.x * blockDim.x + threadIdx.x;
    if (i < n) { parent[i] = (int)i; size[i] = 0; }
}
template <int MODE>
__global__ __launch_bounds__(256) void k_groups_edges(DParams prm, int* parent, int2* edges, int* nedges, int cap) {
    const int64_t id = (int64_t)blockIdx.x * 4 + (threadIdx.x >> 6);
    const int lane = (int)(threadIdx.x & 63u);
    if (id >= prm.pool_n) return;
    const DPatch* p = prm.pool + id;
    if (!(p->flags & 1)) return;
    const PGeo me = load_geo(p);
    const DView* vw = prm.views + me.ref;
    unsigned long long listed = 0ull;
    if (MODE == 1) {
        for (int i = 0; i < min(p->nimages, MVS_LISTCAP); ++i) listed |= 1ull << p->images[i];
        for (int i = 0; i < min(p->nvimages, MVS_LISTCAP); ++i) listed |= 1ull << p->vimages[i];
    }
    int gx, gy;
    cell_of(prm, vw, me.coord, gx, gy);
    csr_off_t lstart = 0;
    int ln = 0;
    if (lane < 18) {
        const int kind = lane / 9, yt = gy + (lane % 9) / 3 - 1, xt = gx + lane % 3 - 1;
        if (!(yt < 0 || vw->gh <= yt || xt < 0 || vw->gw <= xt)) {
            const int g = vw->cell_base + yt * vw->gw + xt;
            lstart = kind == 0 ? prm.csr_start[g] : prm.vcsr_start[g];
            ln = kind == 0 ? prm.csr_cnt[g] : prm.vcsr_cnt[g];
        }
    }
    int before = ln;
    for (int d = 1; d < 32; d <<= 1) { const int o = __shfl_up(before, d); if (lane >= d) before += o; }
    const int total = __builtin_amdgcn_readlane(before, 17);
    before -= ln;
    int myroot = -1;
    auto entry_at = [&](int k, int& eid) -> bool {
        int lo = 0;
#pragma unroll
        for (int step = 16; step >= 1; step >>= 1) { const int pc = __shfl(before, lo + step); if (pc <= k) lo += step; }
        const int l_first = __shfl(before, lo);
        const csr_off_t l_start = __shfl(lstart, lo);
        if (k >= total) return false;
        eid = (lo >= 9 ? prm.vcsr_id32 : prm.csr_id32)[l_start + (k - l_first)];
        return true;
    };
    auto edge = [&](const int eid) {
        if (eid == (int)id) return;
        if (MODE != 2 && __atomic_load_n(&parent[eid], __ATOMIC_RELAXED) == __atomic_load_n(&parent[id], __ATOMIC_RELAXED)) return;
        if (!(prm.pool[eid].flags & 1)) return;
        const PGeo q = load_geo(prm.pool + eid);
        if (!is_neighbor(prm, me, q, 1.0f )) return;
        if (MODE == 0) uf_union(parent, (int)id, eid);
        else if (MODE == 1) {
            if (!((listed >> q.ref) & 1ull)) return;
            const DView* qw = prm.views + q.ref;
            int px, py, qx, qy;
            cell_of(prm, qw, me.coord, px, py);
            cell_of(prm, qw, q.coord, qx, qy);
            if (px < 0 || qw->gw <= px || py < 0 || qw->gh <= py) return;
            if (abs(px - qx) <= 1 && abs(py - qy) <= 1) uf_union(parent, (int)id, eid);
        } else {
            if (myroot < 0) myroot = uf_find(parent, (int)id);
            const int rq = uf_find(parent, eid);
            if (rq != myroot) {
                const int k2 = atomicAdd(nedges, 1);
                if (k2 < cap) edges[k2] = make_int2(myroot, rq);
            }
        }
    };
    for (int k0 = 0; k0 < total; k0 += 128) {
        int e0 = -1, e1 = -1;
        const bool h0 = entry_at(k0 + lane, e0), h1 = entry_at(k0 + 64 + lane, e1);
        if (h0) edge(e0);
        if (h1) edge(e1);
    }
}
__global__ void k_groups_count(DParams prm, int* parent, int* size, int sat) {
    const int64_t id = (int64_t)blockIdx.x * blockDim.x + threadIdx.x;
    if (id >= prm.pool_n || !(prm.pool[id].flags & 1)) return;
    const int r = uf_find(parent, (int)id);
    parent[id] = r;
    const int r0 = __builtin_amdgcn_readfirstlane(r);
    const unsigned long long same = __ballot(r == r0);
    if (r == r0) { if ((int)(threadIdx.x & 63u) == __ffsll((long long)same) - 1 && __atomic_load_n(&size[r0], __ATOMIC_RELAXED) < sat) atomicAdd(&size[r0], (int)__popcll(same)); }
    else if (__atomic_load_n(&size[r], __ATOMIC_RELAXED) < sat) atomicAdd(&size[r], 1);
}
__global__ void k_groups_kill(DParams prm, const int* parent, const int* size, int threshold, uint8_t* kill) {
    const int64_t id = (int64_t)blockIdx.x * blockDim.x + threadIdx.x;
    if (id >= prm.pool_n || !(prm.pool[id].flags & 1)) return;
    if (size[parent[id]] < threshold) kill[id] = 1;
}

void mvsk_fill_ncc(const DParams& prm, unsigned long long* evals, hipStream_t st) {
    if (prm.pool_n > 0) hipLaunchKernelGGL(k_fill_ncc, dim3((unsigned)((prm.pool_n + 63) / 64)), dim3(64), MVS_FRAME_LDS_BYTES, st, prm, evals);
}
void mvsk_kill_count(const uint8_t* kill, int64_t n, int32_t* cnt, hipStream_t st) { if (n > 0) hipLaunchKernelGGL(k_kill_count, dim3(nblk(n, 256)), dim3(256), 0, st, kill, n, cnt); }
void mvsk_kill_export(const uint8_t* kill, int64_t n, const int32_t* base, int32_t* ids, int64_t cap, hipStream_t st) {
    if (n > 0) hipLaunchKernelGGL(k_kill_export, dim3(nblk(n, 256)), dim3(256), 0, st, kill, n, base, ids, cap);
}
void mvsk_apply_kill_flags(DPatch* pool, uint8_t* kill, int64_t n, hipStream_t st) { if (n > 0) hipLaunchKernelGGL(k_apply_kill_flags, dim3(nblk(n, 256)), dim3(256), 0, st, pool, kill, n); }
void mvsk_apply_kill_ids(DPatch* pool, const int32_t* ids, int64_t n, int64_t pool_n, hipStream_t st) {
    if (n > 0) hipLaunchKernelGGL(k_apply_kill_ids, dim3(nblk(n, 256)), dim3(256), 0, st, pool, ids, n, pool_n);
}
void mvsk_append_records(DPatch* pool, int64_t pool_n, const DPatch* recs, int64_t n, hipStream_t st) {
    if (n > 0) hipLaunchKernelGGL(k_append_records, dim3(nblk(n, 256)), dim3(256), 0, st, pool, pool_n, recs, n);
}
void mvsk_alive_count(const DPatch* pool, int64_t n, int32_t* cnt, hipStream_t st) { if (n > 0) hipLaunchKernelGGL(k_alive_count, dim3(nblk(n, 256)), dim3(256), 0, st, pool, n, cnt); }
void mvsk_alive_gather(const DPatch* pool, int64_t n, const int32_t* base, DPatch* out, int64_t cap, hipStream_t st) {
    if (n > 0) hipLaunchKernelGGL(k_alive_gather, dim3(nblk(n, 256)), dim3(256), 0, st, pool, n, base, out, cap);
}
void mvsk_filter_vimages(const DParams& prm, int additive, int64_t first, int64_t last, const uint32_t* dirty, hipStream_t st) {
    if (last <= first) return;
    const int gl = std::max(prm.nviews <= 16 ? 16 : (prm.nviews <= 32 ? 32 : 64), (int)MVS_LISTCAP);
    const unsigned nb = (unsigned)((last - first + 64 / gl - 1) / (64 / gl));
    if (gl == 16) hipLaunchKernelGGL(k_filter_vimages<16>, dim3(nb), dim3(64), 0, st, prm, additive, first, last, dirty);
    else if (gl == 32) hipLaunchKernelGGL(k_filter_vimages<32>, dim3(nb), dim3(64), 0, st, prm, additive, first, last, dirty);
    else hipLaunchKernelGGL(k_filter_vimages<64>, dim3(nb), dim3(64), 0, st, prm, additive, first, last, dirty);
}
void mvsk_geo_pack(const DPatch* pool, int64_t n, float4* geo, uint8_t* ref, int* bad, hipStream_t st) {
    if (n <= 0) return;
    hipLaunchKernelGGL(k_geo_pack, dim3((unsigned)((n + 255) / 256)), dim3(256), 0, st, pool, n, geo, ref, bad);
}
void mvsk_filter_outside(const DParams& prm, uint8_t* kill, int64_t first, int64_t last, hipStream_t st) {
    if (last > first) hipLaunchKernelGGL(k_filter_outside, dim3((unsigned)(last - first)), dim3(64), 0, st, prm, kill, first);
}
size_t mvsk_texs_lds_bytes(const DParams& prm) {
    const size_t texs = texs_gram_lds_bytes(prm);
    return texs > (size_t)MVS_FRAME_LDS_BYTES ? texs : (size_t)MVS_FRAME_LDS_BYTES;
}
void mvsk_filter_exact(const DParams& prm, uint8_t* kill, unsigned long long* evals, unsigned long long* stage, int64_t first, int64_t last, hipStream_t st) {
    if (last > first) hipLaunchKernelGGL(k_filter_exact, dim3((unsigned)((last - first + MVS_FE_PATCHES - 1) / MVS_FE_PATCHES)), dim3(64), mvsk_texs_lds_bytes(prm), st, prm, kill, evals, stage, first, last);
}
void mvsk_filter_neighbor(const DParams& prm, uint8_t* kill, int32_t* retry, int32_t* nretry, int32_t* overflow, unsigned long long* stats, int64_t first, int64_t last, hipStream_t st) {
    if (last <= first) return;
    hipLaunchKernelGGL((k_filter_neighbor<MVS_FILTER_HASH_CAP, MVS_FILTER_ROW_CAP>), dim3((unsigned)(last - first)), dim3(64),
                       (size_t)(MVS_SET_LDS_FLOATS(MVS_FILTER_HASH_CAP, MVS_FILTER_ROW_CAP) + 64) * sizeof(float), st, prm, kill, (const int32_t*)nullptr, 0, retry, nretry, overflow, stats, first);
}
void mvsk_filter_neighbor_retry(const DParams& prm, uint8_t* kill, const int32_t* todo, int32_t ntodo, int32_t* overflow, unsigned long long* stats, hipStream_t st) {
    if (ntodo <= 0) return;
    hipLaunchKernelGGL((k_filter_neighbor<MVS_FILTER2_HASH_CAP, MVS_FILTER2_ROW_CAP>), dim3((unsigned)ntodo), dim3(64),
                       (size_t)MVS_SET_LDS_FLOATS(MVS_FILTER2_HASH_CAP, MVS_FILTER2_ROW_CAP) * sizeof(float), st, prm, kill, todo, ntodo, (int32_t*)nullptr, (int32_t*)nullptr, overflow, stats, (int64_t)0);
}
void mvsk_groups(const DParams& prm, int* parent, int* size, int threshold, uint8_t* kill, hipStream_t st) {
    if (prm.pool_n <= 0) return;
    hipLaunchKernelGGL(k_groups_init, dim3(nblk(prm.pool_n, 256)), dim3(256), 0, st, parent, size, prm.pool_n);
    hipLaunchKernelGGL(k_groups_edges<0>, dim3(nblk(prm.pool_n, 4)), dim3(256), 0, st, prm, parent, (int2*)nullptr, (int*)nullptr, 0);
    hipLaunchKernelGGL(k_groups_count, dim3(nblk(prm.pool_n, 256)), dim3(256), 0, st, prm, parent, size, threshold);
    hipLaunchKernelGGL(k_groups_kill, dim3(nblk(prm.pool_n, 256)), dim3(256), 0, st, prm, parent, size, threshold, kill);
}
void mvsk_groups_literal_edges(const DParams& prm, int* parent, int* size, int* edges2, int* nedges, int cap, hipStream_t st) {
    if (prm.pool_n <= 0) return;
    hipLaunchKernelGGL(k_groups_init, dim3(nblk(prm.pool_n, 256)), dim3(256), 0, st, parent, size, prm.pool_n);
    hipLaunchKernelGGL(k_groups_edges<1>, dim3(nblk(prm.pool_n, 4)), dim3(256), 0, st, prm, parent, (int2*)nullptr, (int*)nullptr, 0);
    hipLaunchKernelGGL(k_groups_count, dim3(nblk(prm.pool_n, 256)), dim3(256), 0, st, prm, parent, size, INT_MAX);
    hipLaunchKernelGGL(k_groups_edges<2>, dim3(nblk(prm.pool_n, 4)), dim3(256), 0, st, prm, parent, reinterpret_cast<int2*>(edges2), nedges, cap);
}
void mvsk_groups_kill(const DParams& prm, const int* parent, const int* size, int threshold, uint8_t* kill, hipStream_t st) {
    if (prm.pool_n > 0) hipLaunchKernelGGL(k_groups_kill, dim3(nblk(prm.pool_n, 256)), dim3(256), 0, st, prm, parent, size, threshold, kill);
}
```

### mvskit_amd/csrc/mvs_index.hip

```cpp
#include <hip/hip_runtime.h>
#include <algorithm>
#include "mvs_camera.cuh"
#include "mvs_common.cuh"
#include "mvs_kernels.h"

using namespace mvsdev;

__device__ __forceinline__ unsigned long long list_key(float ncc, int64_t id) {
    return ((unsigned long long)(~sortable_f32(ncc + 0.0f)) << 32) | (unsigned long long)(uint32_t)id;
}
__global__ void k_index_count(DParams prm, int32_t* __restrict__ cnt, int32_t* __restrict__ vcnt, unsigned long long* __restrict__ total) {
    const int64_t id = (int64_t)blockIdx.x * blockDim.x + threadIdx.x;
    int mine = 0;
    if (id < prm.pool_n && (prm.pool[id].flags & 1)) {
        const DPatch* p = prm.pool + id;
        const F4 coord = ld4(p->coord);
        const int n = cnt ? min(p->nimages, MVS_LISTCAP) : 0;
        for (int i = 0; i < n; ++i) {
            const DView* vw = prm.views + p->images[i];
            int ix, iy;
            cell_of(prm, vw, coord, ix, iy);
            if (ix < 0 || vw->gw <= ix || iy < 0 || vw->gh <= iy) continue;
            atomicAdd(&cnt[vw->cell_base + iy * vw->gw + ix], 1);
            ++mine;
        }
        if (vcnt) {
            const int nv = min(p->nvimages, MVS_LISTCAP);
            for (int i = 0; i < nv; ++i) {
                const DView* vw = prm.views + p->vimages[i];
                int ix, iy;
                cell_of(prm, vw, coord, ix, iy);
                if (ix < 0 || vw->gw <= ix || iy < 0 || vw->gh <= iy) continue;
                atomicAdd(&vcnt[vw->cell_base + iy * vw->gw + ix], 1);
                ++mine;
            }
        }
    }
    for (int d = 32; d >= 1; d >>= 1) mine += __shfl_xor(mine, d);
    if (total && (threadIdx.x & 63) == 0 && mine) atomicAdd(total, (unsigned long long)mine);
}
__global__ void k_index_fill(DParams prm, int vgrid, const csr_off_t* __restrict__ start, int32_t* __restrict__ cursor, unsigned long long* __restrict__ ids) {
    const int64_t id = (int64_t)blockIdx.x * blockDim.x + threadIdx.x;
    if (id >= prm.pool_n) return;
    const DPatch* p = prm.pool + id;
    if (!(p->flags & 1)) return;
    const F4 coord = ld4(p->coord);
    const unsigned long long key = list_key(p->ncc, id);
    const int n = vgrid ? min(p->nvimages, MVS_LISTCAP) : min(p->nimages, MVS_LISTCAP);
    for (int i = 0; i < n; ++i) {
        const DView* vw = prm.views + (vgrid ? p->vimages[i] : p->images[i]);
        int ix, iy;
        cell_of(prm, vw, coord, ix, iy);
        if (ix < 0 || vw->gw <= ix || iy < 0 || vw->gh <= iy) continue;
        const int g = vw->cell_base + iy * vw->gw + ix;
        ids[start[g] + atomicAdd(&cursor[g], 1)] = key;
    }
}
__global__ void k_index_fill_direct(DParams prm, int vgrid, const csr_off_t* __restrict__ start, int32_t* __restrict__ cursor, int32_t* __restrict__ id32) {
    const int64_t id = (int64_t)blockIdx.x * blockDim.x + threadIdx.x;
    if (id >= prm.pool_n) return;
    const DPatch* p = prm.pool + id;
    if (!(p->flags & 1)) return;
    const F4 coord = ld4(p->coord);
    const int n = vgrid ? min(p->nvimages, MVS_LISTCAP) : min(p->nimages, MVS_LISTCAP);
    for (int i = 0; i < n; ++i) {
        const DView* vw = prm.views + (vgrid ? p->vimages[i] : p->images[i]);
        int ix, iy;
        cell_of(prm, vw, coord, ix, iy);
        if (ix < 0 || vw->gw <= ix || iy < 0 || vw->gh <= iy) continue;
        const int g = vw->cell_base + iy * vw->gw + ix;
        const csr_off_t slot = start[g] + atomicAdd(&cursor[g], 1);
        id32[slot] = (int32_t)id;
    }
}
__global__ void k_index_sort_trim(DParams prm, const csr_off_t* __restrict__ start, unsigned long long* __restrict__ ids, int do_trim,
                                  unsigned long long* __restrict__ trimmed) {
    const int g = blockIdx.x * blockDim.x + threadIdx.x;
    const bool in = g < prm.total_cells;
    const csr_off_t b = in ? start[g] : 0, e = in ? start[g + 1] : 0;
    for (csr_off_t i = b + 1; i < e; ++i) {
        const unsigned long long k = ids[i];
        csr_off_t j = i - 1;
        while (j >= b) {
            const unsigned long long o = ids[j];
            if (o < k) break;
            ids[j + 1] = o;
            --j;
        }
        ids[j + 1] = k;
    }
    if (do_trim) {
        int mine = 0;
        for (csr_off_t k = b + prm.cap; k < e; ++k) {
            const int old = atomicAnd(&prm.pool[(uint32_t)ids[k]].flags, ~1);
            mine += old & 1;
        }
        for (int d = 32; d >= 1; d >>= 1) mine += __shfl_xor(mine, d);
        if ((threadIdx.x & 63) == 0 && mine) atomicAdd(trimmed + (blockIdx.x & 255u), (unsigned long long)mine);
    }
}
__global__ void k_index_finalize(DParams prm, int vgrid, const csr_off_t* __restrict__ start, unsigned long long* __restrict__ ids,
                                 int32_t* __restrict__ id32, int32_t* __restrict__ cnt_alive) {
    const int g = blockIdx.x * blockDim.x + threadIdx.x;
    if (g >= prm.total_cells) return;
    const csr_off_t b = start[g], e = start[g + 1];
    int n = 0;
    for (csr_off_t k = b; k < e; ++k) {
        const int id = (int)(uint32_t)ids[k];
        const DPatch* p = prm.pool + id;
        if (!(p->flags & 1)) continue;
        if (!vgrid) ids[b + n] = ((unsigned long long)(uint32_t)p->images[0] << 32) | (unsigned long long)__float_as_uint(p->ncc);
        id32[b + n] = id;
        ++n;
    }
    cnt_alive[g] = n;
}
__global__ void k_index_pack(DParams prm, const csr_off_t* __restrict__ start, const csr_off_t* __restrict__ start2, const int32_t* __restrict__ cnt_alive,
                             const unsigned long long* __restrict__ ids, const int32_t* __restrict__ id32_in, ListKey* __restrict__ key, int32_t* __restrict__ id32_out) {
    const int g = blockIdx.x * blockDim.x + threadIdx.x;
    if (g >= prm.total_cells) return;
    const csr_off_t b = start[g], b2 = start2[g];
    const int n = cnt_alive[g];
    for (int k = 0; k < n; ++k) {
        id32_out[b2 + k] = id32_in[b + k];
        if (key) {
            const unsigned long long w = ids[b + k];
            ListKey lk;
            lk.ncc = __uint_as_float((uint32_t)w); lk.ref = (int32_t)(w >> 32);
            key[b2 + k] = lk;
        }
    }
}
__global__ __launch_bounds__(256) void k_depth_maps(DParams prm, unsigned long long* __restrict__ dp, const uint32_t* __restrict__ dirty) {
    const int64_t id = (int64_t)blockIdx.x * 64 + (threadIdx.x & 63u);
    if (id >= prm.pool_n) return;
    const DPatch* p = prm.pool + id;
    if (!(p->flags & 1)) return;
    const F4 coord = ld4(p->coord);
    for (int image = (int)(threadIdx.x >> 6); image < prm.nviews; image += 4) {
        const DView* vw = prm.views + image;
        const F3 ic = project(vw, coord, prm.level);
        const float fx = ic.x / (float)prm.csize, fy = ic.y / (float)prm.csize;
        const int xs[2] = {(int)floorf(fx), (int)ceilf(fx)}, ys[2] = {(int)floorf(fy), (int)ceilf(fy)};
        const float depth = dot4(ld4(vw->oaxis), coord);
        const unsigned long long key = ((unsigned long long)sortable_f32(depth) << 32) | (unsigned long long)(uint32_t)id;
        for (int j = 0; j < 2; ++j) for (int i = 0; i < 2; ++i) {
            if (xs[i] < 0 || vw->gw <= xs[i] || ys[j] < 0 || vw->gh <= ys[j]) continue;
            if (i == 1 && xs[1] == xs[0]) continue;
            if (j == 1 && ys[1] == ys[0]) continue;
            const int cell = vw->cell_base + ys[j] * vw->gw + xs[i];
            if (dirty && !((dirty[cell >> 5] >> (cell & 31)) & 1u)) continue;
            unsigned long long* cellp = &dp[cell];
            if (key < __builtin_nontemporal_load(cellp)) atomicMin(cellp, key);
        }
    }
}
__global__ __launch_bounds__(256) void k_depth_mark_dirty(DParams prm, const uint8_t* __restrict__ kill, unsigned long long* __restrict__ dp, uint32_t* __restrict__ dirty) {
    const int64_t id = (int64_t)blockIdx.x * 64 + (threadIdx.x & 63u);
    if (id >= prm.pool_n || !kill[id]) return;
    const DPatch* p = prm.pool + id;
    if (!(p->flags & 1)) return;
    const F4 coord = ld4(p->coord);
    for (int image = (int)(threadIdx.x >> 6); image < prm.nviews; image += 4) {
        const DView* vw = prm.views + image;
        const F3 ic = project(vw, coord, prm.level);
        const float fx = ic.x / (float)prm.csize, fy = ic.y / (float)prm.csize;
        const int xs[2] = {(int)floorf(fx), (int)ceilf(fx)}, ys[2] = {(int)floorf(fy), (int)ceilf(fy)};
        for (int j = 0; j < 2; ++j) for (int i = 0; i < 2; ++i) {
            if (xs[i] < 0 || vw->gw <= xs[i] || ys[j] < 0 || vw->gh <= ys[j]) continue;
            if (i == 1 && xs[1] == xs[0]) continue;
            if (j == 1 && ys[1] == ys[0]) continue;
            const int cell = vw->cell_base + ys[j] * vw->gw + xs[i];
            if ((uint32_t)(dp[cell] & 0xffffffffull) != (uint32_t)id) continue;
            dp[cell] = ~0ull;
            atomicOr(&dirty[cell >> 5], 1u << (cell & 31));
        }
    }
}
__global__ void k_best_ncc_map(DParams prm, int view, unsigned long long* __restrict__ best) {
    const int64_t id = (int64_t)blockIdx.x * blockDim.x + threadIdx.x;
    if (id >= prm.pool_n) return;
    const DPatch* p = prm.pool + id;
    if (!(p->flags & 1) || p->nimages == 0 || p->images[0] != view) return;
    const DView* vw = prm.views + view;
    int ix, iy;
    cell_of(prm, vw, ld4(p->coord), ix, iy);
    if (ix < 0 || vw->gw <= ix || iy < 0 || vw->gh <= iy) return;
    const unsigned long long key = ((unsigned long long)sortable_f32(p->ncc) << 32) | (unsigned long long)(0xffffffffu - (uint32_t)id);
    atomicMax(&best[iy * vw->gw + ix], key);
}
__global__ void k_map_extract(DParams prm, int view, int kind, const unsigned long long* __restrict__ sel, float* __restrict__ depth,
                              float* __restrict__ normal, int32_t* __restrict__ ids, int ncells) {
    const int c = blockIdx.x * blockDim.x + threadIdx.x;
    if (c >= ncells) return;
    const unsigned long long k = sel[c];
    const bool empty = kind == 0 ? (k == ~0ull) : (k == 0ull);
    if (empty) {
        depth[c] = __int_as_float(0x7fc00000);
        normal[3 * c] = normal[3 * c + 1] = normal[3 * c + 2] = __int_as_float(0x7fc00000);
        ids[c] = -1;
        return;
    }
    const uint32_t id = kind == 0 ? (uint32_t)(k & 0xffffffffull) : 0xffffffffu - (uint32_t)(k & 0xffffffffull);
    const DPatch* p = prm.pool + id;
    depth[c] = dot4(ld4((prm.views + view)->oaxis), ld4(p->coord));
    normal[3 * c] = p->normal[0]; normal[3 * c + 1] = p->normal[1]; normal[3 * c + 2] = p->normal[2];
    ids[c] = (int32_t)id;
}

void mvsk_index_count(const DParams& prm, int32_t* cnt, int32_t* vcnt, unsigned long long* total, hipStream_t st) {
    if (prm.pool_n > 0) hipLaunchKernelGGL(k_index_count, dim3(nblk(prm.pool_n, 256)), dim3(256), 0, st, prm, cnt, vcnt, total);
}
void mvsk_index_fill(const DParams& prm, int vgrid, const csr_off_t* start, int32_t* cursor, unsigned long long* ids, hipStream_t st) {
    if (prm.pool_n > 0) hipLaunchKernelGGL(k_index_fill, dim3(nblk(prm.pool_n, 256)), dim3(256), 0, st, prm, vgrid, start, cursor, ids);
}
void mvsk_index_fill_direct(const DParams& prm, int vgrid, const csr_off_t* start, int32_t* cursor, int32_t* id32, hipStream_t st) {
    if (prm.pool_n > 0) hipLaunchKernelGGL(k_index_fill_direct, dim3(nblk(prm.pool_n, 256)), dim3(256), 0, st, prm, vgrid, start, cursor, id32);
}
void mvsk_index_sort_trim(const DParams& prm, const csr_off_t* start, unsigned long long* ids, int do_trim, unsigned long long* trimmed, hipStream_t st) {
    hipLaunchKernelGGL(k_index_sort_trim, dim3(nblk(prm.total_cells, 256)), dim3(256), 0, st, prm, start, ids, do_trim, trimmed);
}
void mvsk_index_finalize(const DParams& prm, int vgrid, const csr_off_t* start, unsigned long long* ids, int32_t* id32, int32_t* cnt_alive, hipStream_t st) {
    hipLaunchKernelGGL(k_index_finalize, dim3(nblk(prm.total_cells, 256)), dim3(256), 0, st, prm, vgrid, start, ids, id32, cnt_alive);
}
void mvsk_index_pack(const DParams& prm, const csr_off_t* start, const csr_off_t* start2, const int32_t* cnt_alive, const unsigned long long* ids, const int32_t* id32_in,
                     ListKey* key, int32_t* id32_out, hipStream_t st) {
    hipLaunchKernelGGL(k_index_pack, dim3(nblk(prm.total_cells, 256)), dim3(256), 0, st, prm, start, start2, cnt_alive, ids, id32_in, key, id32_out);
}
void mvsk_depth_maps(const DParams& prm, unsigned long long* dp, const uint32_t* dirty, hipStream_t st) {
    if (prm.pool_n > 0) hipLaunchKernelGGL(k_depth_maps, dim3(nblk(prm.pool_n, 64)), dim3(256), 0, st, prm, dp, dirty);
}
void mvsk_depth_mark_dirty(const DParams& prm, const uint8_t* kill, unsigned long long* dp, uint32_t* dirty, hipStream_t st) {
    if (prm.pool_n > 0) hipLaunchKernelGGL(k_depth_mark_dirty, dim3(nblk(prm.pool_n, 64)), dim3(256), 0, st, prm, kill, dp, dirty);
}
void mvsk_best_ncc_map(const DParams& prm, int view, unsigned long long* best, hipStream_t st) {
    if (prm.pool_n > 0) hipLaunchKernelGGL(k_best_ncc_map, dim3(nblk(prm.pool_n, 256)), dim3(256), 0, st, prm, view, best);
}
void mvsk_map_extract(const DParams& prm, int view, int kind, const unsigned long long* sel, float* depth, float* normal, int32_t* ids, int ncells, hipStream_t st) {
    hipLaunchKernelGGL(k_map_extract, dim3(nblk(ncells, 256)), dim3(256), 0, st, prm, view, kind, sel, depth, normal, ids, ncells);
}
```

### mvskit_amd/csrc/mvs_kernels.h

```cpp
#pragma once
#include <hip/hip_runtime.h>
#include "mvs_types.h"

void mvsk_rgb_to_rgba(const uint8_t* rgb, uint32_t* out, int64_t n, hipStream_t st);
void mvsk_rgba_to_rgb(const uint32_t* in, uint8_t* rgb, int64_t n, hipStream_t st);
void mvsk_pyr_down(const uint32_t* src, int pw, int ph, uint32_t* dst, int w, int h, hipStream_t st);
void mvsk_mask_down(const uint8_t* src, int pw, int ph, uint8_t* dst, int w, int h, hipStream_t st);
void mvsk_mask_binarise(uint8_t* m, int64_t n, hipStream_t st);
void mvsk_exclusive_scan(const int32_t* in, int32_t* out, int64_t n, int32_t* tmp, hipStream_t st);
void mvsk_exclusive_scan_off(const int32_t* in, csr_off_t* out, int64_t n, csr_off_t* tmp, hipStream_t st);
void mvsk_gather_i32(const int32_t* src, const int32_t* idx, int32_t* out, int64_t n, hipStream_t st);
void mvsk_scatter_i32(int32_t* dst, const int32_t* idx, const int32_t* val, int64_t n, hipStream_t st);
void mvsk_index_count(const DParams& prm, int32_t* cnt, int32_t* vcnt, unsigned long long* total, hipStream_t st);
void mvsk_index_fill(const DParams& prm, int vgrid, const csr_off_t* start, int32_t* cursor, unsigned long long* ids, hipStream_t st);
void mvsk_index_fill_direct(const DParams& prm, int vgrid, const csr_off_t* start, int32_t* cursor, int32_t* id32, hipStream_t st);
void mvsk_index_sort_trim(const DParams& prm, const csr_off_t* start, unsigned long long* ids, int do_trim, unsigned long long* trimmed, hipStream_t st);
void mvsk_index_finalize(const DParams& prm, int vgrid, const csr_off_t* start, unsigned long long* ids, int32_t* id32, int32_t* cnt_alive, hipStream_t st);
void mvsk_index_pack(const DParams& prm, const csr_off_t* start, const csr_off_t* start2, const int32_t* cnt_alive, const unsigned long long* ids, const int32_t* id32_in,
                     ListKey* key, int32_t* id32_out, hipStream_t st);
void mvsk_depth_maps(const DParams& prm, unsigned long long* dp, const uint32_t* dirty, hipStream_t st);
void mvsk_depth_mark_dirty(const DParams& prm, const uint8_t* kill, unsigned long long* dp, uint32_t* dirty, hipStream_t st);
void mvsk_best_ncc_map(const DParams& prm, int view, unsigned long long* best, hipStream_t st);
void mvsk_map_extract(const DParams& prm, int view, int kind, const unsigned long long* sel, float* depth, float* normal, int32_t* ids, int ncells, hipStream_t st);
struct RefineSel { int simplex; int max_evals; float xtol; };
struct KernelVariant { bool launched, full_window, narrow, pair; };
KernelVariant mvsk_kernel_variant(const DParams& prm);
size_t mvsk_sweep_lds_bytes(const DParams& prm);
KernelVariant mvsk_sweep(const DParams& prm, const SweepArgs& a, const RefineSel& rs, hipStream_t st);
void mvsk_sweep_retry(const DParams& prm, const SweepArgs& a, int nretry, const RefineSel& rs, hipStream_t st);
void mvsk_job_work(const DParams& prm, const SweepArgs& a, int mode, int shift, int32_t* work, hipStream_t st);
int mvsk_job_list_seg(const SweepArgs& a);
void mvsk_job_list(const DParams& prm, const SweepArgs& a, int32_t* flags, int32_t* scan, int32_t* scan_tmp, int32_t* list, int32_t* bounds, hipStream_t st);
void mvsk_job_cuts(const int32_t* scan, int64_t njobs, int n, int32_t* cuts, hipStream_t st);
void mvsk_commit_count(const SweepArgs& a, int32_t* cnt, hipStream_t st);
void mvsk_commit_copy(const SweepArgs& a, const int32_t* base, DPatch* dst, int64_t dst_cap, int32_t* per_view, int keep_key, hipStream_t st);
void mvsk_fill_ncc(const DParams& prm, unsigned long long* evals, hipStream_t st);
void mvsk_kill_count(const uint8_t* kill, int64_t n, int32_t* cnt, hipStream_t st);
void mvsk_kill_export(const uint8_t* kill, int64_t n, const int32_t* base, int32_t* ids, int64_t cap, hipStream_t st);
void mvsk_apply_kill_flags(DPatch* pool, uint8_t* kill, int64_t n, hipStream_t st);
void mvsk_apply_kill_ids(DPatch* pool, const int32_t* ids, int64_t n, int64_t pool_n, hipStream_t st);
void mvsk_append_records(DPatch* pool, int64_t pool_n, const DPatch* recs, int64_t n, hipStream_t st);
void mvsk_alive_count(const DPatch* pool, int64_t n, int32_t* cnt, hipStream_t st);
void mvsk_alive_gather(const DPatch* pool, int64_t n, const int32_t* base, DPatch* out, int64_t cap, hipStream_t st);
void mvsk_filter_vimages(const DParams& prm, int additive, int64_t first, int64_t last, const uint32_t* dirty, hipStream_t st);
void mvsk_geo_pack(const DPatch* pool, int64_t n, float4* geo, uint8_t* ref, int* bad, hipStream_t st);
void mvsk_filter_outside(const DParams& prm, uint8_t* kill, int64_t first, int64_t last, hipStream_t st);
void mvsk_filter_exact(const DParams& prm, uint8_t* kill, unsigned long long* evals, unsigned long long* stage, int64_t first, int64_t last, hipStream_t st);
void mvsk_filter_neighbor(const DParams& prm, uint8_t* kill, int32_t* retry, int32_t* nretry, int32_t* overflow, unsigned long long* stats, int64_t first, int64_t last, hipStream_t st);
void mvsk_filter_neighbor_retry(const DParams& prm, uint8_t* kill, const int32_t* todo, int32_t ntodo, int32_t* overflow, unsigned long long* stats, hipStream_t st);
void mvsk_groups(const DParams& prm, int* parent, int* size, int threshold, uint8_t* kill, hipStream_t st);
void mvsk_groups_literal_edges(const DParams& prm, int* parent, int* size, int* edges2, int* nedges, int cap, hipStream_t st);
void mvsk_groups_kill(const DParams& prm, const int* parent, const int* size, int threshold, uint8_t* kill, hipStream_t st);
KernelVariant mvsk_probe(const DParams& prm, int op, int64_t n, const DPatch* in, const float* in_f, DPatch* out, float* out_f, int32_t* out_i, const RefineSel& rs,
                         hipStream_t st);
void mvsk_ply_select(const DPatch* pool, const int32_t* base, int64_t i0, int64_t i1, int32_t* idx, hipStream_t st);
void mvsk_ply_colour(const DPatch* pool, const int32_t* idx, int64_t n, const DView* views, int nviews, int level, int ascii, uint32_t* rgb, int32_t* len,
                     hipStream_t st);
void mvsk_ply_emit(const DPatch* pool, const int32_t* idx, int64_t n, const uint32_t* rgb, const int64_t* off, uint8_t* out, hipStream_t st);
struct SeedView { float P[12]; int32_t W, H, view; };
struct SeedCam { float center[4]; float ipscale; };
void mvsk_seed_accumulate(const SeedView& sv, const float* map, const uint8_t* mask, const float* xyz, int64_t n, float* sum, unsigned long long* bits,
                          hipStream_t st);
void mvsk_seed_flags(const SeedCam* cams, int level, const float* xyz, const float* sum, const unsigned long long* bits, int64_t n, int32_t* keep,
                     hipStream_t st);
void mvsk_seed_emit(const SeedCam* cams, int nviews, int level, float thr, float tmp_unit, const float* xyz, const float* sum, const unsigned long long* bits,
                    const int32_t* keep, const int32_t* base, int64_t n, DPatch* dst, hipStream_t st);
struct SeedRandomArgs { SeedChainArgs chain; uint32_t seed; float max_tilt; int32_t view; float dmin, dmax; };
size_t mvsk_texs_lds_bytes(const DParams& prm);
void mvsk_seed_random_hypotheses(const DParams& prm, const SeedRandomArgs& a, int64_t ncells, const int32_t* cells, DPatch* out, hipStream_t st);
void mvsk_seed_random(const DParams& prm, const SeedRandomArgs& a, int ncells, DPatch* stage, int32_t* keep, hipStream_t st);
void mvsk_seed_gather(const DPatch* stage, const int32_t* keep, const int32_t* base, int n, DPatch* dst, int32_t id0, hipStream_t st);
void mvsk_seed_points_hypotheses(const DParams& prm, int K, int64_t n, const float* xyz, DPatch* out, int32_t* count, hipStream_t st);
void mvsk_seed_points(const DParams& prm, const SeedPointsArgs& a, const float* xyz, DPatch* stage, int32_t* keep, hipStream_t st);
void mvsk_depth_ranges(const DParams& prm, int64_t n, const float* xyz, uint32_t* lo, uint32_t* hi, unsigned long long* cnt, hipStream_t st);
struct MapsArgs { int64_t pix_base[MVS_MAXVIEWS + 1]; float depth_tol, normal_cos; };
void mvsk_maps_select(const DParams& prm, unsigned long long* sel, hipStream_t st);
void mvsk_maps_render(const DParams& prm, int view, int W, int H, int source, const unsigned long long* sel, int32_t* ids, float* pts, hipStream_t st);
void mvsk_maps_agree(const DParams& prm, const MapsArgs& a, int view, int64_t npix, const int32_t* ids, const float* pts, unsigned long long* agree,
                     float* depth, float* normal, float* conf, hipStream_t st);
void mvsk_maps_flag(int64_t npix, int view, const int32_t* ids, const unsigned long long* agree, int min_consistent, int dedupe, int32_t* flag,
                    uint8_t* flag8, hipStream_t st);
void mvsk_maps_expand(int64_t npix, const uint8_t* flag8, int32_t* flag, hipStream_t st);
void mvsk_maps_gather(const DParams& prm, int view, int64_t npix, const int32_t* ids, const float* pts, const int32_t* flag, const int32_t* base,
                      void* out, int64_t cap, hipStream_t st);
struct MeshVol { float origin[3]; float voxel; int32_t nx, ny, nz; float trunc; int32_t min_count; };
inline int64_t mesh_npoints(const MeshVol& vol) { return (int64_t)vol.nx * vol.ny * vol.nz; }
void mvsk_mesh_tsdf(const DParams& prm, const MapsArgs& a, const MeshVol& vol, const int32_t* ids, const uint8_t* usable, float* tsdf, int32_t* count,
                    hipStream_t st);
void mvsk_mesh_state(const MeshVol& vol, const float* tsdf, const int32_t* count, uint8_t* state, hipStream_t st);
void mvsk_mesh_edges(const MeshVol& vol, const uint8_t* state, uint8_t* mask, int32_t* cnt, hipStream_t st);
void mvsk_mesh_verts(const MeshVol& vol, const float* tsdf, const uint8_t* mask, const int32_t* vbase, float* verts, int64_t cap_v, hipStream_t st);
void mvsk_mesh_tcount(const MeshVol& vol, const uint8_t* state, int32_t* cnt, hipStream_t st);
void mvsk_mesh_tris(const MeshVol& vol, const uint8_t* state, const uint8_t* mask, const int32_t* vbase, const int64_t* tbase, int32_t* tris,
                    int64_t cap_t, hipStream_t st);
void mvsk_mesh_normals_scan(int64_t n_v, const float* verts, int64_t n_t, const int32_t* tris, uint32_t* mbits, uint32_t* bad, hipStream_t st);
void mvsk_mesh_normals_accum(const float* verts, int64_t n_t, const int32_t* tris, const uint32_t* mbits, long long* acc, hipStream_t st);
void mvsk_mesh_normals_finish(int64_t n_v, const long long* acc, float* normals, hipStream_t st);
struct MeshColourArgs { float occl_tol, min_cos; };
void mvsk_mesh_colours(const DParams& prm, const MapsArgs& a, const MeshColourArgs& m, int64_t n_v, const float* verts, const float* normals,
                       const int32_t* ids, const uint8_t* usable, uint8_t* rgb, uint8_t* used, hipStream_t st);
void mvsk_mesh_colours_visible(const DParams& prm, const MapsArgs& a, const MeshColourArgs& m, int64_t n_v, const float* verts, const float* normals,
                               const int32_t* ids, const uint8_t* usable, const unsigned long long* visible, uint8_t* rgb, uint8_t* used, hipStream_t st);
void mvsk_mrender_project(const DParams& prm, int view, int64_t n_v, const float* verts, int32_t* scr, float* vd, uint32_t* ok, hipStream_t st);
void mvsk_mrender_raster(int64_t n_t, const int32_t* tris, const int32_t* scr, const float* vd, const uint32_t* ok, int W, int H, int small_max,
                         unsigned long long* keys, int32_t* list, unsigned long long* counts, hipStream_t st);
void mvsk_mrender_resolve(int64_t npix, const unsigned long long* keys, float* depth, int32_t* tri, unsigned long long* covered, hipStream_t st);
void mvsk_mrender_visible(int view, float tol, int64_t n_v, const int32_t* scr, const float* vd, const uint32_t* ok, int W, int H, const unsigned long long* keys,
                          unsigned long long* visible, hipStream_t st);
void mvsk_mesh_check_ids(int64_t n_v, int64_t n_t, const int32_t* tris, uint32_t* bad, hipStream_t st);
void mvsk_mesh_components(int64_t n_v, int64_t n_t, const int32_t* tris, int32_t* parent, int32_t* size, unsigned long long* ncomp, hipStream_t st);
void mvsk_mesh_flatten(int64_t n_v, int32_t* parent, hipStream_t st);
void mvsk_mesh_largest(int64_t n_v, const int32_t* parent, const int32_t* size, unsigned long long* best, hipStream_t st);
void mvsk_mesh_keep(int64_t n_t, const int32_t* tris, const int32_t* parent, const int32_t* size, int64_t min_triangles, int largest_only,
                    const unsigned long long* best, int32_t* tflag, int32_t* vflag, hipStream_t st);
void mvsk_mesh_gather(int64_t n_v, const float* verts, int32_t* vflag, const int32_t* vbase, float* out_verts, int64_t cap_v, int64_t n_t, const int32_t* tris,
                      const int32_t* tflag, const int32_t* tbase, int32_t* out_tris, int64_t cap_t, hipStream_t st);
void mvsk_mesh_smooth_step(int64_t n_v, const float* xin, float* xout, float f, int64_t n_t, const int32_t* tris, uint32_t* mbits, long long* acc, int32_t* cnt,
                           hipStream_t st);
void mvsk_mdec_members(int64_t n_v, const float* verts, int64_t n_t, const int32_t* tris, const float* origin, float cell, int32_t* used,
                       unsigned long long* key, uint32_t* mbits, uint32_t* bad, hipStream_t st);
void mvsk_mdec_table(int64_t n, const unsigned long long* key, unsigned long long* tkey, int32_t* tval, int64_t slots, int32_t* out, uint32_t* fail,
                     hipStream_t st);
void mvsk_mdec_tkey1(int64_t n_t, const int32_t* tris, const int32_t* rep, unsigned long long* key, hipStream_t st);
void mvsk_mdec_tkey2(int64_t n_t, const int32_t* tris, const int32_t* rep, const int32_t* first, unsigned long long* key, hipStream_t st);
void mvsk_mdec_keep(int64_t n_t, const int32_t* tris, const int32_t* rep, const int32_t* winner, int32_t* tflag, int32_t* vflag, hipStream_t st);
void mvsk_mdec_positions(int placement, int64_t n_v, const float* verts, const int32_t* rep, const int32_t* vflag, const int32_t* vbase, const uint32_t* mbits,
                         long long* acc, int32_t* cnt, unsigned long long* best, float* out_verts, int64_t cap_v, hipStream_t st);
void mvsk_mdec_gather(int64_t n_v, const int32_t* rep, const int32_t* vflag, const int32_t* vbase, int32_t* vmap, int64_t n_t, const int32_t* tris,
                      const int32_t* tflag, const int32_t* tbase, int32_t* out_tris, int64_t cap_t, hipStream_t st);
void mvsk_mfill_boundaries(int64_t n_v, int64_t n_t, const int32_t* tris, unsigned long long* tkey, int32_t* tval, int64_t slots, int32_t* parent, int32_t* outc,
                           int32_t* inc, int32_t* cplx, int32_t* next, int32_t* hed, int32_t* rbad, int32_t* loop, int32_t* length, unsigned long long* counts,
                           uint32_t* fail, hipStream_t st);
void mvsk_mfill_plan(int64_t n_v, const float* verts, const int32_t* loop, const int32_t* length, int32_t max_edges, int32_t* tcnt, int32_t* vcnt, uint32_t* mbits,
                     uint32_t* bad, unsigned long long* nfilled, hipStream_t st);
void mvsk_mfill_emit(int64_t n_v, const float* verts, const int32_t* loop, const int32_t* length, int32_t max_edges, const int32_t* next, const int32_t* tbase,
                     const int32_t* vbase, const uint32_t* mbits, long long* acc, int32_t* add_tris, int64_t cap_t, float* add_verts, int64_t cap_v, hipStream_t st);
```

Baseline: 33.39 million.

## Overlap index builds on side streams and compact unscored NCC fill into a list

Runs the visibility-grid list build and the depth-map build on two auxiliary streams, forked after the main list's trim step, so they overlap with the main list finalize and pack. The NCC fill now launches only over a compacted list of unscored patches collected during the count kernel, instead of scanning the whole pool. A side array holding alive bit and key is added so finalize avoids reading full patch records. The sweep-retry count readback is folded into the single post-sweep sync. Together these aim to cut serialized kernel time and host syncs, at the cost of extra memory, more synchronization events and more complex ordering.

New measurement: 33.68 million, median of 6. No clear change (+0.9%).

```diff
diff --git a/mvskit_amd/csrc/mvs_engine.cpp b/mvskit_amd/csrc/mvs_engine.cpp
--- a/mvskit_amd/csrc/mvs_engine.cpp
+++ b/mvskit_amd/csrc/mvs_engine.cpp
@@ -209,6 +209,9 @@
     hipError_t he = hipStreamCreate(&e->stream);
     if (he != hipSuccess) { g_err = std::string("hipStreamCreate: ") + hipGetErrorString(he); delete e; return MVS_ERR_HIP; }
     for (auto& ev : e->ev) (void)hipEventCreate(&ev);
+    for (auto& s : e->aux) if ((he = hipStreamCreate(&s)) != hipSuccess) break;
+    for (hipEvent_t* ev : {&e->fork_ev, &e->join_ev[0], &e->join_ev[1]}) if (he == hipSuccess) he = hipEventCreateWithFlags(ev, hipEventDisableTiming);
+    if (he != hipSuccess) { g_err = std::string("mvs_engine_create: side streams: ") + hipGetErrorString(he); mvs_engine_destroy(e); return MVS_ERR_HIP; }
     for (auto& ev : e->fev) (void)hipEventCreate(&ev);
     if (e->misc.ensure(misc::words) || e->counters.ensure(MVS_COUNTER_SLOTS) || e->error_flag.ensure(1)) { delete e; return MVS_ERR_HIP; }
     (void)hipMemset(e->misc.p, 0, misc::words * sizeof(unsigned long long));
@@ -221,7 +224,10 @@
     if (!e) return MVS_OK;
     (void)hipSetDevice(e->cfg.device);
     (void)hipStreamSynchronize(e->stream);
+    for (auto& s : e->aux) if (s) (void)hipStreamSynchronize(s);
     (void)mvs_engine_comm_release(e);
+    for (hipEvent_t ev : {e->fork_ev, e->join_ev[0], e->join_ev[1]}) if (ev) (void)hipEventDestroy(ev);
+    for (auto& s : e->aux) if (s) (void)hipStreamDestroy(s);
     for (auto& ev : e->ev) if (ev) (void)hipEventDestroy(ev);
     for (auto& ev : e->fev) if (ev) (void)hipEventDestroy(ev);
     (void)hipStreamDestroy(e->stream);
@@ -308,7 +314,7 @@
         size_t free_b = 0, total_b = 0;
         if (hipMemGetInfo(&free_b, &total_b) == hipSuccess && total_b > 0) {
             pool_cap = std::max<int64_t>(std::min<int64_t>(pool_cap, (int64_t)(total_b / 6 / sizeof(DPatch))), std::min<int64_t>(pool_cap, nc));
-            const double per_patch = 2.5 * (double)sizeof(DPatch) + 17.0;
+            const double per_patch = 2.5 * (double)sizeof(DPatch) + 25.0;
             const int64_t fit = (int64_t)(0.6 * (double)free_b / per_patch);
             if (fit < pool_cap) pool_cap = std::max<int64_t>(fit, std::min<int64_t>(pool_cap, nc / 4 + 1024));
         }
@@ -329,6 +335,7 @@
     if (e->uf_parent.ensure(pool_cap) || e->uf_size.ensure(pool_cap) || e->dirty.ensure((nc + 31) / 32 + 1) || e->fstat_buf.ensure(fstat::words)) return MVS_ERR_HIP;
     if (e->staging.ensure(std::max<int64_t>(pool_cap / 2, 1024))) return MVS_ERR_HIP;
     if (e->tmp_rec_out.ensure(16)) return MVS_ERR_HIP;
+    if (e->side.ensure(pool_cap) || e->scan_tmp_aux.ensure(nc / 256 + 4096)) return MVS_ERR_HIP;
     HIPCHK(hipStreamSynchronize(st));
     e->pool_n = 0;
     e->have_views = true;
@@ -510,7 +517,7 @@
     if (n == 0) return MVS_OK;
     HIPCHK(hipSetDevice(e->cfg.device));
     hipStream_t st = e->stream;
-    if (op == MVS_PROBE_POSTPROCESS && e->prm.depth > 0) if (int r = build_index(e, nullptr)) return r;
+    if (op == MVS_PROBE_POSTPROCESS && e->prm.depth > 0) if (int r = build_index(e)) return r;
     const int64_t nf_out = op == MVS_PROBE_MATH ? 5 * n : ((op == MVS_PROBE_REFINE || op == MVS_PROBE_REFINE_X) && rs.simplex ? 4 * n : n);
     if (e->tmp_rec_in.ensure(n) || e->tmp_rec_out.ensure(n) || e->tmp_f_in.ensure(n) || e->tmp_f_out.ensure(nf_out) || e->tmp_i.ensure(n + 1)) return MVS_ERR_HIP;
     if (op == MVS_PROBE_MATH) {
diff --git a/mvskit_amd/csrc/mvs_engine_impl.h b/mvskit_amd/csrc/mvs_engine_impl.h
--- a/mvskit_amd/csrc/mvs_engine_impl.h
+++ b/mvskit_amd/csrc/mvs_engine_impl.h
@@ -60,6 +60,7 @@
 namespace misc {
 constexpr int stage_counter = 0;
 constexpr int fill_evals = 1;
+constexpr int unscored = 3;
 constexpr int neighbor_retry = 4;
 constexpr int sweep_retry = 5;
 constexpr int geo_bad = 6;
@@ -117,6 +118,8 @@
     mvs_refiner refiner{MVS_REFINE_HALVING, 500, 1e-4f};
     DParams prm{};
     hipStream_t stream = nullptr;
+    hipStream_t aux[2] = {nullptr, nullptr};
+    hipEvent_t fork_ev = nullptr, join_ev[2] = {nullptr, nullptr};
     bool have_views = false;
     std::vector<DView> hviews;
     DevBuf<DView> dviews;
@@ -133,6 +136,8 @@
     DevBuf<csr_off_t> start_raw;
     DevBuf<int32_t> id32_raw;
     DevBuf<int64_t> scan_tmp;
+    DevBuf<int64_t> scan_tmp_aux;
+    DevBuf<unsigned long long> side;
     DevBuf<unsigned long long> ids;
     DevBuf<ListKey> key;
     DevBuf<int32_t> id32, vid32;
@@ -193,20 +198,25 @@
 int need_state(const mvs_engine* e, Need need, const char* who);
 int scan_total(mvs_engine* e, const int32_t* flags, int32_t* base, int32_t* scan, int64_t n, int64_t* count);
 
-int build_list(mvs_engine* e, bool vgrid, bool trim, bool unordered = false);
-int build_depth(mvs_engine* e);
-int build_index(mvs_engine* e, unsigned long long* trimmed_out);
+struct BuildLane { hipStream_t st; int64_t* scan_tmp; };
+inline BuildLane main_lane(mvs_engine* e) { return BuildLane{e->stream, e->scan_tmp.p}; }
+int build_list(mvs_engine* e, bool vgrid, bool trim, bool unordered, BuildLane lane, hipEvent_t after_trim = nullptr, bool score = false);
+inline int build_list(mvs_engine* e, bool vgrid, bool trim, bool unordered = false) { return build_list(e, vgrid, trim, unordered, main_lane(e)); }
+int build_depth(mvs_engine* e, hipStream_t st);
+inline int build_depth(mvs_engine* e) { return build_depth(e, e->stream); }
+int build_index(mvs_engine* e);
 enum class Count { alive, kills, apply_kills };
 int count_pool(mvs_engine* e, Count what, int64_t* total);
 int ensure_counts(mvs_engine* e);
 int compact_pool(mvs_engine* e);
 void discard_pass(mvs_engine* e);
 
-template <typename T> int read_back(mvs_engine* e, const T* dev, T* host) {
-    HIPCHK(hipMemcpyAsync(host, dev, sizeof(T), hipMemcpyDeviceToHost, e->stream));
-    HIPCHK(hipStreamSynchronize(e->stream));
+template <typename T> int read_back(hipStream_t st, const T* dev, T* host) {
+    HIPCHK(hipMemcpyAsync(host, dev, sizeof(T), hipMemcpyDeviceToHost, st));
+    HIPCHK(hipStreamSynchronize(st));
     return MVS_OK;
 }
+template <typename T> int read_back(mvs_engine* e, const T* dev, T* host) { return read_back(e->stream, dev, host); }
 
 template <typename Apply> int commit_pool(mvs_engine* e, Apply&& apply) {
     hipStream_t st = e->stream;
diff --git a/mvskit_amd/csrc/mvs_engine_pass.cpp b/mvskit_amd/csrc/mvs_engine_pass.cpp
--- a/mvskit_amd/csrc/mvs_engine_pass.cpp
+++ b/mvskit_amd/csrc/mvs_engine_pass.cpp
@@ -9,8 +9,8 @@
 
 namespace mvseng {
 
-int build_list(mvs_engine* e, bool vgrid, bool trim, bool unordered) {
-    hipStream_t st = e->stream;
+int build_list(mvs_engine* e, bool vgrid, bool trim, bool unordered, BuildLane lane, hipEvent_t after_trim, bool score) {
+    hipStream_t st = lane.st;
     const int64_t nc = e->total_cells;
     DParams p = current_params(e);
     DevBuf<int32_t>& cnt = vgrid ? e->vcnt : e->cnt;
@@ -19,15 +19,21 @@
     DevBuf<unsigned long long>& ids = e->ids;
     DevBuf<int32_t>& id32 = vgrid ? e->vid32 : e->id32;
     DevBuf<int32_t>& cnt_alive = vgrid ? e->vcnt_alive : e->cnt_alive;
+    const bool direct = unordered && !trim;
+    if (!direct) { if (int r = e->side.ensure(e->pool.cap)) return r; }
     HIPCHK(hipMemsetAsync(cnt.p, 0, (size_t)(nc + 1) * sizeof(int32_t), st));
-    mvsk_index_count(p, vgrid ? nullptr : cnt.p, vgrid ? cnt.p : nullptr, nullptr, st);
-    const bool direct = unordered && !trim;
+    int32_t* const n_unscored = reinterpret_cast<int32_t*>(e->misc.p + misc::unscored);
+    mvsk_index_count(p, vgrid ? nullptr : cnt.p, vgrid ? cnt.p : nullptr, nullptr, score ? e->kill_cnt.p : nullptr, score ? n_unscored : nullptr, st);
     DevBuf<csr_off_t>& raw = e->start_raw;
     csr_off_t* const first_scan = direct ? start.p : raw.p;
-    mvsk_exclusive_scan_off(cnt.p, first_scan, nc, reinterpret_cast<csr_off_t*>(e->scan_tmp.p), st);
+    mvsk_exclusive_scan_off(cnt.p, first_scan, nc, reinterpret_cast<csr_off_t*>(lane.scan_tmp), st);
     csr_off_t tot64 = 0;
-    if (int r = read_back(e, first_scan + nc, &tot64)) return r;
+    int32_t nscore = 0;
+    if (score) HIPCHK(hipMemcpyAsync(&nscore, n_unscored, sizeof nscore, hipMemcpyDeviceToHost, st));
+    if (int r = read_back(st, first_scan + nc, &tot64)) return r;
     const int64_t tot = (int64_t)tot64;
+    if (nscore < 0 || nscore > e->pool_n) { g_err = "build_list: the list of unscored patches is out of range"; return MVS_ERR_STATE; }
+    if (nscore > 0) mvsk_fill_ncc(p, e->kill_cnt.p, nscore, e->misc.p + misc::fill_evals, st);
     if (!unordered) { if (int r = ids.ensure(tot + 16)) return r; }
     if (!vgrid && !unordered) { if (int r = e->key.ensure(tot + 16)) return r; }
     if (int r = id32.ensure(tot + 16)) return r;
@@ -40,36 +46,47 @@
         return MVS_OK;
     }
     if (int r = e->id32_raw.ensure(tot + 16)) return r;
-    mvsk_index_fill(p, vgrid ? 1 : 0, raw.p, cursor.p, ids.p, st);
-    mvsk_index_sort_trim(p, raw.p, ids.p, trim ? 1 : 0, e->misc.p + misc::trim_parts, st);
-    mvsk_index_finalize(p, vgrid ? 1 : 0, raw.p, ids.p, e->id32_raw.p, cnt_alive.p, st);
-    mvsk_exclusive_scan_off(cnt_alive.p, start.p, nc, reinterpret_cast<csr_off_t*>(e->scan_tmp.p), st);
+    mvsk_index_fill(p, vgrid ? 1 : 0, raw.p, cursor.p, ids.p, e->side.p, st);
+    mvsk_index_sort_trim(p, raw.p, ids.p, trim ? 1 : 0, e->misc.p + misc::trim_parts, e->side.p, st);
+    if (after_trim) HIPCHK(hipEventRecord(after_trim, st));
+    mvsk_index_finalize(p, vgrid ? 1 : 0, raw.p, ids.p, e->id32_raw.p, cnt_alive.p, e->side.p, st);
+    mvsk_exclusive_scan_off(cnt_alive.p, start.p, nc, reinterpret_cast<csr_off_t*>(lane.scan_tmp), st);
     mvsk_index_pack(p, raw.p, start.p, cnt_alive.p, ids.p, e->id32_raw.p, vgrid ? nullptr : e->key.p, id32.p, st);
     e->lists_dense[vgrid ? 1 : 0] = true;
     return MVS_OK;
 }
-int build_depth(mvs_engine* e) {
+int build_depth(mvs_engine* e, hipStream_t st) {
     const DParams p = current_params(e);
-    HIPCHK(hipMemsetAsync(e->dpgrid.p, 0xff, (size_t)e->total_cells * sizeof(unsigned long long), e->stream));
-    mvsk_depth_maps(p, e->dpgrid.p, nullptr, e->stream);
-    return MVS_OK;
-}
-int build_index(mvs_engine* e, unsigned long long* trimmed_out) {
-    hipStream_t st = e->stream;
-    const DParams p = current_params(e);
-    HIPCHK(hipMemsetAsync(e->misc.p + misc::fill_evals, 0, 2 * sizeof(unsigned long long), st));
+    HIPCHK(hipMemsetAsync(e->dpgrid.p, 0xff, (size_t)e->total_cells * sizeof(unsigned long long), st));
+    mvsk_depth_maps(p, e->dpgrid.p, nullptr, st);
+    return MVS_OK;
+}
+static int build_index_forked(mvs_engine* e) {
+    HIPCHK(hipStreamWaitEvent(e->aux[1], e->fork_ev, 0));
+    if (int r = build_depth(e, e->aux[1])) return r;
+    HIPCHK(hipEventRecord(e->join_ev[1], e->aux[1]));
+    if (want_vgrid(e)) {
+        HIPCHK(hipStreamWaitEvent(e->aux[0], e->fork_ev, 0));
+        if (int r = build_list(e, true, false, true, BuildLane{e->aux[0], e->scan_tmp_aux.p})) return r;
+        HIPCHK(hipEventRecord(e->join_ev[0], e->aux[0]));
+        HIPCHK(hipStreamWaitEvent(e->stream, e->join_ev[0], 0));
+    }
+    HIPCHK(hipStreamWaitEvent(e->stream, e->join_ev[1], 0));
+    return MVS_OK;
+}
+int build_index(mvs_engine* e) {
+    hipStream_t st = e->stream;
+    static_assert(misc::unscored == misc::fill_evals + 2, "fill_evals[2] and unscored are cleared together");
+    HIPCHK(hipMemsetAsync(e->misc.p + misc::fill_evals, 0, 3 * sizeof(unsigned long long), st));
     HIPCHK(hipMemsetAsync(e->misc.p + misc::trim_parts, 0, misc::trim_nparts * sizeof(unsigned long long), st));
-    mvsk_fill_ncc(p, e->misc.p + misc::fill_evals, st);
     e->ncc_dirty = false;
-    if (int r = build_list(e, false, true)) return r;
-    if (want_vgrid(e)) if (int r = build_list(e, true, false, true)) return r;
-    if (int r = build_depth(e)) return r;
-    if (trimmed_out) {
-        unsigned long long part[misc::trim_nparts];
-        HIPCHK(hipMemcpyAsync(part, e->misc.p + misc::trim_parts, sizeof part, hipMemcpyDeviceToHost, st));
-        HIPCHK(hipStreamSynchronize(st));
-        *trimmed_out = 0;
-        for (unsigned long long v : part) *trimmed_out += v;
+    if (int r = e->scan_tmp_aux.ensure(e->total_cells / 256 + 4096)) return r;
+    if (int r = build_list(e, false, true, false, main_lane(e), e->fork_ev, true)) return r;
+    if (int r = build_index_forked(e)) {
+        const std::string keep = g_err;
+        (void)hipStreamSynchronize(e->aux[0]); (void)hipStreamSynchronize(e->aux[1]); (void)hipStreamSynchronize(st);
+        g_err = keep;
+        return r;
     }
     HIPCHK(hipGetLastError());
     return MVS_OK;
@@ -122,6 +139,7 @@
     return MVS_OK;
 }
 
+
 void discard_pass(mvs_engine* e) {
     if (e->kill.p && e->pool_n > 0) (void)hipMemsetAsync(e->kill.p, 0, (size_t)e->pool_n, e->stream);
     (void)hipStreamSynchronize(e->stream);
@@ -153,10 +171,9 @@
     HIPCHK(hipSetDevice(e->cfg.device));
     hipStream_t st = e->stream;
     HIPCHK(hipEventRecord(e->ev[0], st));
-    unsigned long long trimmed = 0;
     {
         Range rg("mvs:index");
-        if (int r = build_index(e, &trimmed)) return r;
+        if (int r = build_index(e)) return r;
     }
     SweepArgs& a = e->sa;
     memset(&a, 0, sizeof a);
@@ -229,23 +246,31 @@
     const KernelVariant sweep_kernel = mvsk_sweep(p, a, rs, st);
     if (sweep_kernel.launched) { e->sweep_kernels[sweep_kernel.full_window ? 1 : 0] += 1; e->sampler_launches[sweep_kernel.narrow ? 1 : 0] += 1; }
     e->pass_retried = 0;
-    if (want_vgrid(e)) {
-        int32_t nretry = 0;
-        if (int r = read_back(e, a.nretry, &nretry)) return r;
-        e->pass_retried = nretry;
-        if (nretry > 0) { mvsk_sweep_retry(p, a, nretry, rs, st); e->retried_cells += nretry; }
-    }
     HIPCHK(hipEventRecord(e->ev[2], st));
     std::vector<DCounters> hcs(MVS_COUNTER_SLOTS);
-    int32_t herr = 0;
+    int32_t herr = 0, nretry = 0;
     unsigned long long fill[2] = {0, 0};
+    unsigned long long trim_part[misc::trim_nparts];
     HIPCHK(hipMemcpyAsync(fill, e->misc.p + misc::fill_evals, sizeof fill, hipMemcpyDeviceToHost, st));
+    HIPCHK(hipMemcpyAsync(trim_part, e->misc.p + misc::trim_parts, sizeof trim_part, hipMemcpyDeviceToHost, st));
+    HIPCHK(hipMemcpyAsync(&nretry, a.nretry, sizeof nretry, hipMemcpyDeviceToHost, st));
     HIPCHK(hipMemcpyAsync(hcs.data(), e->counters.p, hcs.size() * sizeof(DCounters), hipMemcpyDeviceToHost, st));
     HIPCHK(hipMemcpyAsync(&herr, e->error_flag.p, sizeof herr, hipMemcpyDeviceToHost, st));
     int32_t hbounds[MVS_SWEEP_QUEUES + 1];
     HIPCHK(hipMemcpyAsync(hbounds, list_bounds, sizeof hbounds, hipMemcpyDeviceToHost, st));
     HIPCHK(hipStreamSynchronize(st));
+    if (want_vgrid(e) && nretry > 0) {
+        e->pass_retried = nretry;
+        mvsk_sweep_retry(p, a, nretry, rs, st);
+        e->retried_cells += nretry;
+        HIPCHK(hipEventRecord(e->ev[2], st));
+        HIPCHK(hipMemcpyAsync(hcs.data(), e->counters.p, hcs.size() * sizeof(DCounters), hipMemcpyDeviceToHost, st));
+        HIPCHK(hipMemcpyAsync(&herr, e->error_flag.p, sizeof herr, hipMemcpyDeviceToHost, st));
+        HIPCHK(hipStreamSynchronize(st));
+    }
     HIPCHK(hipGetLastError());
+    unsigned long long trimmed = 0;
+    for (unsigned long long v : trim_part) trimmed += v;
     mvs_counters sum{};
     for (const DCounters& c : hcs) {
         add_counters(sum, c);
diff --git a/mvskit_amd/csrc/mvs_filter.cuh b/mvskit_amd/csrc/mvs_filter.cuh
--- a/mvskit_amd/csrc/mvs_filter.cuh
+++ b/mvskit_amd/csrc/mvs_filter.cuh
@@ -7,16 +7,10 @@
 
 using namespace mvsdev;
 
-__global__ __launch_bounds__(64) void k_fill_ncc(DParams prm, unsigned long long* evals) {
+__global__ __launch_bounds__(64) void k_fill_ncc(DParams prm, const int32_t* __restrict__ list, int n, unsigned long long* evals) {
     WaveCtx wc = make_wave_ctx(prm);
-    const int64_t mine = (int64_t)blockIdx.x * 64 + wc.lane;
-    bool need = false;
-    if (mine < prm.pool_n) need = (prm.pool[mine].flags & 1) && (prm.pool[mine].ncc < 0.0f);
-    unsigned long long todo = ballot(need);
-    while (todo) {
-        const int l = __ffsll((long long)todo) - 1;
-        todo &= todo - 1ull;
-        DPatch* p = prm.pool + ((int64_t)blockIdx.x * 64 + l);
+    for (int k = blockIdx.x; k < n; k += gridDim.x) {
+        DPatch* p = prm.pool + list[k];
         Cand c;
         load_cand(p, wc, c);
         const float ncc = compute_ncc(prm, wc, c.coord, c.normal, c.img, c.nimg);
@@ -401,8 +395,8 @@
     if (size[parent[id]] < threshold) kill[id] = 1;
 }
 
-void mvsk_fill_ncc(const DParams& prm, unsigned long long* evals, hipStream_t st) {
-    if (prm.pool_n > 0) hipLaunchKernelGGL(k_fill_ncc, dim3((unsigned)((prm.pool_n + 63) / 64)), dim3(64), MVS_FRAME_LDS_BYTES, st, prm, evals);
+void mvsk_fill_ncc(const DParams& prm, const int32_t* list, int64_t n, unsigned long long* evals, hipStream_t st) {
+    if (n > 0) hipLaunchKernelGGL(k_fill_ncc, dim3((unsigned)std::min<int64_t>(n, 8192)), dim3(64), MVS_FRAME_LDS_BYTES, st, prm, list, (int)n, evals);
 }
 void mvsk_kill_count(const uint8_t* kill, int64_t n, int32_t* cnt, hipStream_t st) { if (n > 0) hipLaunchKernelGGL(k_kill_count, dim3(nblk(n, 256)), dim3(256), 0, st, kill, n, cnt); }
 void mvsk_kill_export(const uint8_t* kill, int64_t n, const int32_t* base, int32_t* ids, int64_t cap, hipStream_t st) {
diff --git a/mvskit_amd/csrc/mvs_index.hip b/mvskit_amd/csrc/mvs_index.hip
--- a/mvskit_amd/csrc/mvs_index.hip
+++ b/mvskit_amd/csrc/mvs_index.hip
@@ -9,10 +9,27 @@
 __device__ __forceinline__ unsigned long long list_key(float ncc, int64_t id) {
     return ((unsigned long long)(~sortable_f32(ncc + 0.0f)) << 32) | (unsigned long long)(uint32_t)id;
 }
-__global__ void k_index_count(DParams prm, int32_t* __restrict__ cnt, int32_t* __restrict__ vcnt, unsigned long long* __restrict__ total) {
+#define MVS_SIDE_ALIVE (1ull << 32)
+__device__ __forceinline__ unsigned long long side_word(const DPatch* p) {
+    return ((unsigned long long)(uint32_t)p->images[0] << 33) | MVS_SIDE_ALIVE | (unsigned long long)__float_as_uint(p->ncc);
+}
+__global__ void k_index_count(DParams prm, int32_t* __restrict__ cnt, int32_t* __restrict__ vcnt, unsigned long long* __restrict__ total,
+                              int32_t* __restrict__ unscored, int32_t* __restrict__ n_unscored) {
     const int64_t id = (int64_t)blockIdx.x * blockDim.x + threadIdx.x;
     int mine = 0;
-    if (id < prm.pool_n && (prm.pool[id].flags & 1)) {
+    const bool alive = id < prm.pool_n && (prm.pool[id].flags & 1);
+    if (unscored) {
+        const bool need = alive && prm.pool[id].ncc < 0.0f;
+        const unsigned long long todo = __ballot(need);
+        if (todo) {
+            const int lane = (int)(threadIdx.x & 63u);
+            int base = 0;
+            if (lane == 0) base = atomicAdd(n_unscored, __popcll(todo));
+            base = __shfl(base, 0);
+            if (need) unscored[base + __popcll(todo & ((1ull << lane) - 1ull))] = (int32_t)id;
+        }
+    }
+    if (alive) {
         const DPatch* p = prm.pool + id;
         const F4 coord = ld4(p->coord);
         const int n = cnt ? min(p->nimages, MVS_LISTCAP) : 0;
@@ -39,11 +56,13 @@
     for (int d = 32; d >= 1; d >>= 1) mine += __shfl_xor(mine, d);
     if (total && (threadIdx.x & 63) == 0 && mine) atomicAdd(total, (unsigned long long)mine);
 }
-__global__ void k_index_fill(DParams prm, int vgrid, const csr_off_t* __restrict__ start, int32_t* __restrict__ cursor, unsigned long long* __restrict__ ids) {
-    const int64_t id = (int64_t)blockIdx.x * blockDim.x + threadIdx.x;
-    if (id >= prm.pool_n) return;
-    const DPatch* p = prm.pool + id;
-    if (!(p->flags & 1)) return;
+__global__ void k_index_fill(DParams prm, int vgrid, const csr_off_t* __restrict__ start, int32_t* __restrict__ cursor, unsigned long long* __restrict__ ids,
+                             unsigned long long* __restrict__ side) {
+    const int64_t id = (int64_t)blockIdx.x * blockDim.x + threadIdx.x;
+    if (id >= prm.pool_n) return;
+    const DPatch* p = prm.pool + id;
+    if (!(p->flags & 1)) return;
+    side[id] = side_word(p);
     const F4 coord = ld4(p->coord);
     const unsigned long long key = list_key(p->ncc, id);
     const int n = vgrid ? min(p->nvimages, MVS_LISTCAP) : min(p->nimages, MVS_LISTCAP);
@@ -74,7 +93,7 @@
     }
 }
 __global__ void k_index_sort_trim(DParams prm, const csr_off_t* __restrict__ start, unsigned long long* __restrict__ ids, int do_trim,
-                                  unsigned long long* __restrict__ trimmed) {
+                                  unsigned long long* __restrict__ trimmed, unsigned long long* __restrict__ side) {
     const int g = blockIdx.x * blockDim.x + threadIdx.x;
     const bool in = g < prm.total_cells;
     const csr_off_t b = in ? start[g] : 0, e = in ? start[g + 1] : 0;
@@ -92,7 +111,9 @@
     if (do_trim) {
         int mine = 0;
         for (csr_off_t k = b + prm.cap; k < e; ++k) {
-            const int old = atomicAnd(&prm.pool[(uint32_t)ids[k]].flags, ~1);
+            const uint32_t id = (uint32_t)ids[k];
+            const int old = atomicAnd(&prm.pool[id].flags, ~1);
+            if (old & 1) atomicAnd(&side[id], ~MVS_SIDE_ALIVE);
             mine += old & 1;
         }
         for (int d = 32; d >= 1; d >>= 1) mine += __shfl_xor(mine, d);
@@ -100,16 +121,16 @@
     }
 }
 __global__ void k_index_finalize(DParams prm, int vgrid, const csr_off_t* __restrict__ start, unsigned long long* __restrict__ ids,
-                                 int32_t* __restrict__ id32, int32_t* __restrict__ cnt_alive) {
+                                 int32_t* __restrict__ id32, int32_t* __restrict__ cnt_alive, const unsigned long long* __restrict__ side) {
     const int g = blockIdx.x * blockDim.x + threadIdx.x;
     if (g >= prm.total_cells) return;
     const csr_off_t b = start[g], e = start[g + 1];
     int n = 0;
     for (csr_off_t k = b; k < e; ++k) {
         const int id = (int)(uint32_t)ids[k];
-        const DPatch* p = prm.pool + id;
-        if (!(p->flags & 1)) continue;
-        if (!vgrid) ids[b + n] = ((unsigned long long)(uint32_t)p->images[0] << 32) | (unsigned long long)__float_as_uint(p->ncc);
+        const unsigned long long w = side[(uint32_t)id];
+        if (!(w & MVS_SIDE_ALIVE)) continue;
+        if (!vgrid) ids[b + n] = ((w >> 33) << 32) | (w & 0xffffffffull);
         id32[b + n] = id;
         ++n;
     }
@@ -208,20 +229,22 @@
     ids[c] = (int32_t)id;
 }
 
-void mvsk_index_count(const DParams& prm, int32_t* cnt, int32_t* vcnt, unsigned long long* total, hipStream_t st) {
-    if (prm.pool_n > 0) hipLaunchKernelGGL(k_index_count, dim3(nblk(prm.pool_n, 256)), dim3(256), 0, st, prm, cnt, vcnt, total);
-}
-void mvsk_index_fill(const DParams& prm, int vgrid, const csr_off_t* start, int32_t* cursor, unsigned long long* ids, hipStream_t st) {
-    if (prm.pool_n > 0) hipLaunchKernelGGL(k_index_fill, dim3(nblk(prm.pool_n, 256)), dim3(256), 0, st, prm, vgrid, start, cursor, ids);
+void mvsk_index_count(const DParams& prm, int32_t* cnt, int32_t* vcnt, unsigned long long* total, int32_t* unscored, int32_t* n_unscored, hipStream_t st) {
+    if (prm.pool_n > 0) hipLaunchKernelGGL(k_index_count, dim3(nblk(prm.pool_n, 256)), dim3(256), 0, st, prm, cnt, vcnt, total, unscored, n_unscored);
+}
+void mvsk_index_fill(const DParams& prm, int vgrid, const csr_off_t* start, int32_t* cursor, unsigned long long* ids, unsigned long long* side, hipStream_t st) {
+    if (prm.pool_n > 0) hipLaunchKernelGGL(k_index_fill, dim3(nblk(prm.pool_n, 256)), dim3(256), 0, st, prm, vgrid, start, cursor, ids, side);
 }
 void mvsk_index_fill_direct(const DParams& prm, int vgrid, const csr_off_t* start, int32_t* cursor, int32_t* id32, hipStream_t st) {
     if (prm.pool_n > 0) hipLaunchKernelGGL(k_index_fill_direct, dim3(nblk(prm.pool_n, 256)), dim3(256), 0, st, prm, vgrid, start, cursor, id32);
 }
-void mvsk_index_sort_trim(const DParams& prm, const csr_off_t* start, unsigned long long* ids, int do_trim, unsigned long long* trimmed, hipStream_t st) {
-    hipLaunchKernelGGL(k_index_sort_trim, dim3(nblk(prm.total_cells, 256)), dim3(256), 0, st, prm, start, ids, do_trim, trimmed);
-}
-void mvsk_index_finalize(const DParams& prm, int vgrid, const csr_off_t* start, unsigned long long* ids, int32_t* id32, int32_t* cnt_alive, hipStream_t st) {
-    hipLaunchKernelGGL(k_index_finalize, dim3(nblk(prm.total_cells, 256)), dim3(256), 0, st, prm, vgrid, start, ids, id32, cnt_alive);
+void mvsk_index_sort_trim(const DParams& prm, const csr_off_t* start, unsigned long long* ids, int do_trim, unsigned long long* trimmed, unsigned long long* side,
+                          hipStream_t st) {
+    hipLaunchKernelGGL(k_index_sort_trim, dim3(nblk(prm.total_cells, 256)), dim3(256), 0, st, prm, start, ids, do_trim, trimmed, side);
+}
+void mvsk_index_finalize(const DParams& prm, int vgrid, const csr_off_t* start, unsigned long long* ids, int32_t* id32, int32_t* cnt_alive,
+                         const unsigned long long* side, hipStream_t st) {
+    hipLaunchKernelGGL(k_index_finalize, dim3(nblk(prm.total_cells, 256)), dim3(256), 0, st, prm, vgrid, start, ids, id32, cnt_alive, side);
 }
 void mvsk_index_pack(const DParams& prm, const csr_off_t* start, const csr_off_t* start2, const int32_t* cnt_alive, const unsigned long long* ids, const int32_t* id32_in,
                      ListKey* key, int32_t* id32_out, hipStream_t st) {
diff --git a/mvskit_amd/csrc/mvs_kernels.h b/mvskit_amd/csrc/mvs_kernels.h
--- a/mvskit_amd/csrc/mvs_kernels.h
+++ b/mvskit_amd/csrc/mvs_kernels.h
@@ -11,11 +11,13 @@
 void mvsk_exclusive_scan_off(const int32_t* in, csr_off_t* out, int64_t n, csr_off_t* tmp, hipStream_t st);
 void mvsk_gather_i32(const int32_t* src, const int32_t* idx, int32_t* out, int64_t n, hipStream_t st);
 void mvsk_scatter_i32(int32_t* dst, const int32_t* idx, const int32_t* val, int64_t n, hipStream_t st);
-void mvsk_index_count(const DParams& prm, int32_t* cnt, int32_t* vcnt, unsigned long long* total, hipStream_t st);
-void mvsk_index_fill(const DParams& prm, int vgrid, const csr_off_t* start, int32_t* cursor, unsigned long long* ids, hipStream_t st);
+void mvsk_index_count(const DParams& prm, int32_t* cnt, int32_t* vcnt, unsigned long long* total, int32_t* unscored, int32_t* n_unscored, hipStream_t st);
+void mvsk_index_fill(const DParams& prm, int vgrid, const csr_off_t* start, int32_t* cursor, unsigned long long* ids, unsigned long long* side, hipStream_t st);
 void mvsk_index_fill_direct(const DParams& prm, int vgrid, const csr_off_t* start, int32_t* cursor, int32_t* id32, hipStream_t st);
-void mvsk_index_sort_trim(const DParams& prm, const csr_off_t* start, unsigned long long* ids, int do_trim, unsigned long long* trimmed, hipStream_t st);
-void mvsk_index_finalize(const DParams& prm, int vgrid, const csr_off_t* start, unsigned long long* ids, int32_t* id32, int32_t* cnt_alive, hipStream_t st);
+void mvsk_index_sort_trim(const DParams& prm, const csr_off_t* start, unsigned long long* ids, int do_trim, unsigned long long* trimmed, unsigned long long* side,
+                          hipStream_t st);
+void mvsk_index_finalize(const DParams& prm, int vgrid, const csr_off_t* start, unsigned long long* ids, int32_t* id32, int32_t* cnt_alive,
+                         const unsigned long long* side, hipStream_t st);
 void mvsk_index_pack(const DParams& prm, const csr_off_t* start, const csr_off_t* start2, const int32_t* cnt_alive, const unsigned long long* ids, const int32_t* id32_in,
                      ListKey* key, int32_t* id32_out, hipStream_t st);
 void mvsk_depth_maps(const DParams& prm, unsigned long long* dp, const uint32_t* dirty, hipStream_t st);
@@ -34,7 +36,7 @@
 void mvsk_job_cuts(const int32_t* scan, int64_t njobs, int n, int32_t* cuts, hipStream_t st);
 void mvsk_commit_count(const SweepArgs& a, int32_t* cnt, hipStream_t st);
 void mvsk_commit_copy(const SweepArgs& a, const int32_t* base, DPatch* dst, int64_t dst_cap, int32_t* per_view, int keep_key, hipStream_t st);
-void mvsk_fill_ncc(const DParams& prm, unsigned long long* evals, hipStream_t st);
+void mvsk_fill_ncc(const DParams& prm, const int32_t* list, int64_t n, unsigned long long* evals, hipStream_t st);
 void mvsk_kill_count(const uint8_t* kill, int64_t n, int32_t* cnt, hipStream_t st);
 void mvsk_kill_export(const uint8_t* kill, int64_t n, const int32_t* base, int32_t* ids, int64_t cap, hipStream_t st);
 void mvsk_apply_kill_flags(DPatch* pool, uint8_t* kill, int64_t n, hipStream_t st);
```
